# 10XGenomics/supernova

Measured on AMD Instinct MI355X. Metric: Gk-mers/s through count+graph at k=48, 1.2B×150bp; bit-exact counts, higher is better.
Workload: dtype u64

## Files before the change

### include/snk.h

```cpp
#ifndef SNK_H_
#define SNK_H_
#include <stddef.h>
#include <stdint.h>

#ifdef __cplusplus
extern "C" {
#endif

#define SNK_OK 0
#define SNK_E_ARG (-1)
#define SNK_E_HIP (-2)
#define SNK_E_NOGPU (-3)
#define SNK_E_NOMEM (-4)
#define SNK_E_IO (-5)
#define SNK_E_UNSUPPORTED (-6)
#define SNK_E_INTERNAL (-7)

typedef struct snk_ctx snk_ctx;

typedef struct snk_params {
    uint32_t K;
    uint32_t min_qual;
    uint32_t min_freq;
    uint32_t min_bc;
// ... 106 lines not shown
    const void* good_len;
    uint64_t n_kmers;
    const void* keys;
    const void* counts;
    const void* ctx;
    const void* spectrum;
    uint32_t spectrum_bins;
    uint32_t n_circles;
    uint64_t n_unitigs;
    uint64_t unitig_total_bases;
    const void* unitig_off;
    const void* unitig_bases;
    uint32_t rank_rounds;
    uint32_t buckets_split;
    uint32_t max_slots_used;
    uint32_t n_overflow;
    uint64_t scratch_bytes;
    float phase_ms[8];
    float kernel_ms[4];
    uint64_t n_boundary;
    uint64_t n_fragments;
    const void* unitig_group;
    float graph_ms[8];
    uint32_t repartitioned;
    uint32_t n_hot_buckets;
} snk_dev_result;

int snk_dev_count_graph(snk_ctx* ctx, const snk_dev_reads* in, const snk_params* p, snk_dev_result* out, void* stream,
                        char* err, size_t errcap);
int snk_dev_download(snk_ctx* ctx, const void* d_src, void* h_dst, size_t bytes, void* stream);

int snk_dev_stream_begin(snk_ctx* ctx, const snk_params* p, uint32_t read_len, uint64_t total_reads_ub, int has_bc, void* stream, char* err, size_t errcap);
int snk_dev_stream_append(snk_ctx* ctx, const snk_dev_reads* slab, void* stream, char* err, size_t errcap);
int snk_dev_stream_finish(snk_ctx* ctx, snk_dev_result* out, void* stream, char* err, size_t errcap);

uint64_t snk_pack2_bytes(uint64_t n_bases);
int snk_dev_pack2(snk_ctx* ctx, const void* d_bases, uint64_t n_bases, void* d_packed, void* stream);
int snk_dev_unpack2(snk_ctx* ctx, const void* d_packed, uint64_t n_bases, void* d_bases, void* stream);


typedef struct snk_comm snk_comm;
int snk_comm_set_rccl_path(const char* path);
int snk_comm_unique_id(void* id128, char* err, size_t errcap);
int snk_comm_create_rccl(snk_ctx* ctx, const void* id128, uint32_t rank, uint32_t world, snk_comm** out, char* err, size_t errcap);
int snk_comm_from_nccl(snk_ctx* ctx, void* nccl_comm, uint32_t rank, uint32_t world, snk_comm** out, char* err, size_t errcap);
int snk_comm_create_local(uint32_t world, snk_comm** out , char* err, size_t errcap);
typedef int (*snk_comm_a2a_fn)(void* user, const void* send, const uint64_t* sbeg, const uint64_t* scnt, void* recv, const uint64_t* rbeg,
                               const uint64_t* rcnt, uint32_t world);
typedef int (*snk_comm_gather_fn)(void* user, const void* mine, uint32_t k, unsigned long long* all, uint32_t world);
int snk_comm_create_callbacks(uint32_t rank, uint32_t world, snk_comm_a2a_fn a2a, snk_comm_gather_fn gather, void* user, snk_comm** out,
                              char* err, size_t errcap);
int snk_comm_selftest(snk_comm* c, uint64_t seed, uint32_t buckets_per_rank, uint32_t ranges, char* err, size_t errcap);
void snk_comm_destroy(snk_comm* c);
void snk_comm_abort(snk_comm* c);
uint32_t snk_comm_rank(const snk_comm* c);
uint32_t snk_comm_world(const snk_comm* c);
const char* snk_comm_kind(const snk_comm* c);

typedef struct snk_shard_result {
    uint32_t rank, world;
    uint64_t n_reads, n_instances, n_supermers, n_buckets_total;
    uint64_t n_kmers;
    const void* keys;
    const void* counts;
    const void* ctx;
    const void* spectrum;
    uint32_t spectrum_bins, n_circles;
    uint64_t n_unitigs, unitig_total_bases;
    const void* unitig_off;
    const void* unitig_bases;
    const void* unitig_circular;
    uint64_t n_frags, n_frags_total, n_queries, n_link_queries;
    uint64_t exchanged_bytes[8];
    uint32_t host_syncs;
    uint32_t ranking;
    uint32_t buckets_split, max_slots_used;
    float phase_ms[8];
    float join_ms[8];
    float count_kernel_ms;
    uint32_t repartitioned;
    uint32_t n_hot_buckets;
    uint32_t reserved_u;
    uint64_t pair_max_bytes[8];
} snk_shard_result;
uint32_t snk_ctx_last_partition_passes(const snk_ctx* ctx);
uint32_t snk_ctx_last_count_limit(const snk_ctx* ctx);
int snk_shard_step(snk_ctx* ctx, snk_comm* comm, const snk_dev_reads* in, const snk_params* p, uint64_t total_reads, uint32_t flags,
                   snk_shard_result* out, void* stream, char* err, size_t errcap);
int snk_shard_stream_begin(snk_ctx* ctx, snk_comm* comm, const snk_params* p, uint32_t read_len, uint64_t rank_reads_ub, uint64_t total_reads,
                           int has_bc, void* stream, char* err, size_t errcap);
int snk_shard_stream_append(snk_ctx* ctx, const snk_dev_reads* slab, void* stream, char* err, size_t errcap);
int snk_shard_stream_finish(snk_ctx* ctx, snk_comm* comm, uint32_t flags, snk_shard_result* out, void* stream, char* err, size_t errcap);
typedef struct snk_reads {
    uint64_t n_reads;
    uint32_t read_len;
    uint32_t reserved;
    const uint8_t* ascii;
    const uint32_t* rows;
    const uint16_t* lens;
    const uint8_t* quals;
    const uint16_t* good_len;
    const int32_t* bc;
    int64_t ign_bc_below;
} snk_reads;

typedef struct snk_result {
    uint64_t n_instances;
    uint64_t n_kmers;
    uint32_t* kmers;
    uint32_t* counts;
    uint8_t* ctx;
    uint64_t n_unitigs;
    uint64_t* unitig_off;
    uint8_t* unitig_bases;
    uint64_t* spectrum;
    uint32_t spectrum_bins;
    uint32_t reserved;
    float phase_ms[8];
    uint8_t* bv_image;
    uint64_t bv_bytes;
} snk_result;

int snk_count_graph(snk_ctx* ctx, const snk_reads* in, const snk_params* p, snk_result* out, char* err, size_t errcap);
void snk_free(snk_result* r);

int snk_shard_gather_unitigs(snk_ctx* ctx, snk_comm* comm, const snk_shard_result* res, uint32_t K, uint32_t root, uint32_t flags,
                             snk_result* out, void* stream, char* err, size_t errcap);

int snk_host_alloc_pinned(size_t bytes, void** out, char* err, size_t errcap);
void snk_host_free_pinned(void* p);

int snk_write_bv(const char* path, uint64_t n_unitigs, const uint64_t* unitig_off, const uint8_t* unitig_bases,
                 char* err, size_t errcap);
int snk_read_bv(const char* path, uint64_t* n_unitigs, uint64_t** unitig_off, uint8_t** unitig_bases, char* err,
                size_t errcap);

int snk_dev_bv_image(snk_ctx* ctx, uint32_t K, uint64_t n_unitigs, const void* d_unitig_off, const void* d_unitig_bases, int by_first_kmer,
                     const void** d_image, uint64_t* image_bytes, void* stream, char* err, size_t errcap);

typedef struct snk_hbv {
    int32_t n_vertices, n_edges;
    int32_t* v_left;
    int32_t* v_right;
    int32_t* src_unitig;
    uint8_t* is_rc;
    int32_t* fwd_xlat;
    int32_t* rev_xlat;
    int32_t* bvcomp_order;
} snk_hbv;
int snk_hbv_from_unitigs(uint32_t K, uint64_t n_unitigs, const uint64_t* unitig_off, const uint8_t* unitig_bases,
                         snk_hbv* out, char* err, size_t errcap);
uint32_t snk_ctx_last_hbv_flood(const snk_ctx* ctx, uint64_t* device_components, uint64_t* host_components);
uint32_t snk_ctx_last_local_graph(const snk_ctx* ctx, uint64_t* in_chunk_circles, uint32_t* big_chunks);
int snk_dev_hbv(snk_ctx* ctx, uint32_t K, uint64_t n_unitigs, const void* d_unitig_off, const void* d_unitig_bases,
                snk_hbv* out, float* device_ms, void* stream, char* err, size_t errcap);
void snk_hbv_free(snk_hbv* h);
typedef struct snk_dev_paths {
    uint64_t n_reads, n_edges_total;
    const void* offset;
    const void* n_edges;
    const void* start;
    const void* edges;
    uint64_t dict_slots;
    float dict_ms, path_ms;
    const void* unitig_bc_off;
    const void* unitig_bcs;
    uint64_t n_unitig_bcs;
    float bcs_ms;
    uint32_t lookup_index;
    uint64_t n_slow;
    uint32_t retries;
} snk_dev_paths;
#define SNK_PATH_UNITIG_BCS 1u
#define SNK_PATH_UNITIG_BCS_EXHAUSTIVE 2u
#define SNK_PATH_UNITIG_BCS_NOCUT 4u
int snk_dev_path_reads(snk_ctx* ctx, uint32_t K, const snk_dev_reads* in, uint64_t n_unitigs, const void* d_unitig_off, const void* d_unitig_bases,
                       const snk_hbv* h, snk_dev_paths* out, void* stream, char* err, size_t errcap);
int snk_dev_path_reads2(snk_ctx* ctx, uint32_t K, const snk_dev_reads* in, uint64_t n_unitigs, const void* d_unitig_off, const void* d_unitig_bases,
                        const snk_hbv* h, uint32_t flags, snk_dev_paths* out, void* stream, char* err, size_t errcap);
int snk_hbv_involution(const snk_hbv* h, uint64_t n_unitigs, int32_t* inv , char* err, size_t errcap);
int snk_write_hbv(const char* path_hbv, const char* path_inv, uint32_t K, uint64_t n_unitigs, const uint64_t* unitig_off,
                  const uint8_t* unitig_bases, const snk_hbv* h, char* err, size_t errcap);

typedef struct snk_dev_dups {
    uint64_t n_pairs;
    const void* dup;
    uint64_t n_placed;
    uint64_t n_dup_reads;
    uint64_t n_interdup_reads;
    uint64_t n_dup_pairs;
    uint64_t n_art_pairs;
    double interdup_rate;
    float ms;
} snk_dev_dups;
int snk_dev_mark_dups(snk_ctx* ctx, const snk_dev_reads* in, const snk_dev_paths* paths, snk_dev_dups* out, void* stream, char* err, size_t errcap);

typedef struct snk_dev_pidx {
    uint64_t n_hbv_edges, n_entries;
    const void* index_off;
    const void* index_ids;
    const void* counts;
    uint64_t n_empty_edges;
    float ms;
    uint32_t key_bits;
    uint64_t reserved[6];
} snk_dev_pidx;
int snk_dev_paths_index(snk_ctx* ctx, const snk_dev_paths* paths, uint64_t n_hbv_edges, const int32_t* inv, snk_dev_pidx* out, void* stream,
                        char* err, size_t errcap);
int snk_write_paths(const char* path, uint64_t n_reads, const int32_t* offset, const uint32_t* n_edges, const uint64_t* start, const int32_t* edges,
                    char* err, size_t errcap);
int snk_write_paths_index(const char* path_inv, const char* path_countsb, uint64_t n_hbv_edges, const uint64_t* index_off, const uint64_t* index_ids,
                          const int32_t* counts, char* err, size_t errcap);
int snk_write_dup(const char* path, uint64_t n_pairs, const uint8_t* dup, char* err, size_t errcap);

typedef struct snk_dev_pathsx {
    uint64_t n_reads, n_bytes, n_index;
    const void* data;
    const void* index;
    uint64_t n_empty;
    uint64_t n_steps_not_found;
    uint64_t n_offsets_wrapped;
    float ms;
    uint32_t reserved0;
    uint64_t reserved[6];
} snk_dev_pathsx;
int snk_dev_paths_zip(snk_ctx* ctx, const snk_dev_paths* paths, const snk_hbv* h, snk_dev_pathsx* out, void* stream, char* err, size_t errcap);
int snk_dev_paths_unzip(snk_ctx* ctx, const snk_dev_pathsx* in, const snk_hbv* h, snk_dev_paths* out, void* stream, char* err, size_t errcap);
int snk_write_pathsx(const char* path, uint64_t n_reads, const int64_t* index, uint64_t n_index, const uint8_t* data, uint64_t n_bytes, char* err, size_t errcap);
int snk_read_pathsx(const char* path, uint64_t* n_reads, uint64_t* n_index, int64_t** index, uint64_t* n_bytes, uint8_t** data, char* err, size_t errcap);
int snk_write_hbx(const char* path, uint32_t K, uint64_t n_unitigs, const uint64_t* unitig_off, const uint8_t* unitig_bases, const snk_hbv* h, char* err,
                  size_t errcap);

typedef struct snk_dev_extend {
    snk_dev_paths paths;
    uint64_t n_back_extended;
    uint64_t n_cut_to_first;
    uint64_t n_quality_extended;
    uint64_t n_ambiguous;
    uint64_t n_too_many;
    uint64_t n_exact_extended;
    float ms;
    uint32_t reserved0;
    uint64_t n_enumerated;
    uint64_t reserved[5];
} snk_dev_extend;
#define SNK_EXT_BACK 1u
int snk_dev_extend_paths(snk_ctx* ctx, uint32_t K, const snk_dev_reads* in, uint64_t n_unitigs, const void* d_unitig_off, const void* d_unitig_bases,
                         const snk_hbv* h, const snk_dev_paths* paths, uint32_t flags, snk_dev_extend* out, void* stream, char* err, size_t errcap);

#define SNK_BADS_X 1u
typedef struct snk_dev_bads {
    uint64_t n_pairs;
    const void* bad;
    uint64_t n_placed;
    uint64_t n_mismatch_reads;
    uint64_t n_bad_reads;
    uint64_t n_bad_pairs;
    uint64_t n_offsets_wrapped;
    float ms;
    uint32_t n_slabs;
    float tables_ms, kernel_ms;
    uint64_t reserved[5];
} snk_dev_bads;
int snk_dev_mark_bads(snk_ctx* ctx, uint32_t K, const snk_dev_reads* in, uint64_t n_unitigs, const void* d_unitig_off, const void* d_unitig_bases,
                      const snk_hbv* h, const snk_dev_paths* paths, uint32_t flags, snk_dev_bads* out, void* stream, char* err, size_t errcap);
struct snk_df_files;
int snk_dev_mark_bads_df(snk_ctx* ctx, uint32_t K, struct snk_df_files* f, uint64_t first, uint64_t n, uint32_t read_len, uint32_t threads, uint64_t slab_reads,
                         uint64_t n_unitigs, const void* d_unitig_off, const void* d_unitig_bases, const snk_hbv* h, const snk_dev_paths* paths, uint32_t flags,
                         snk_dev_bads* out, char* err, size_t errcap);

#define SNK_HOPS_ONE_GOOD 1u
#define SNK_HOPS_EXT_HOST 2u
typedef struct snk_dev_hops {
    uint64_t n_pairs;
    const void* pairs;
    uint64_t n_part1, n_part2, n_part3;
    uint64_t n_sink_edges;
    uint64_t n_long_edges;
    uint64_t n_two_class;
    uint64_t n_ext_round0;
    uint64_t n_ext_closure;
    uint64_t n_ext_host;
    uint64_t n_not_extended;
    float ms, tables_ms;
    uint32_t ext_budget;
    float part12_ms, part3_ms;
    uint64_t reserved[4];
} snk_dev_hops;
int snk_dev_edge_pairs(snk_ctx* ctx, uint32_t K, uint64_t n_unitigs, const void* d_unitig_off, const void* d_unitig_bases, const snk_hbv* h,
                       const int32_t* inv , const snk_dev_paths* paths, const snk_dev_pidx* px ,
                       const void* d_bc , const void* d_bad , uint32_t flags, uint32_t ext_budget ,
                       snk_dev_hops* out, void* stream, char* err, size_t errcap);
int snk_write_hops(const char* path, uint64_t n_pairs, const int32_t* pairs, char* err, size_t errcap);
int snk_read_hops(const char* path, uint64_t* n_pairs, int32_t** pairs, char* err, size_t errcap);

#define SNK_CLOSE_CG1 1u
#define SNK_CLOSE_PLACE_HOST 2u
typedef struct snk_dev_closures {
    uint64_t n_closures, n_bases, n_pairs;
    const void* closure_off;
    const void* bases;
    const void* pair_first;
    uint64_t n_pairs_0, n_pairs_1, n_pairs_2, n_pairs_many;
    uint64_t n_rows;
    uint64_t n_partners_tried, n_partners_placed;
    uint64_t n_followers;
// ... 267 lines not shown
```

### supernova_amd/csrc/snk_api.hip

```cpp
#include <math.h>
#include <stdlib.h>
#include <execinfo.h>
#include <dlfcn.h>
#include <time.h>

#include <algorithm>

#include "snk_ctx.h"
#include "snk_kernels.h"
#include "snk_synth.h"

static thread_local char g_last_error[512] = "";

hipError_t snk_enter(snk_ctx* ctx) { return hipSetDevice(ctx->device); }

void snk_set_mlen(snk_ctx* ctx, const snk_params* p) {
    uint32_t m = (p->flags & SNK_F_LONG_MINIMISER) ? (uint32_t)SNK_M_LONG : (uint32_t)SNK_M_OF(p->K);
    const unsigned long long v = snk_opt_u64(ctx, SNK_OPT_minimiser_len);
    if (v == SNK_M_LONG || v == SNK_M_OF(p->K)) m = (uint32_t)v;
    ctx->mlen = m;
}

void snk_set_error(char* err, size_t errcap, const char* fmt, ...) {
    va_list ap;
// ... 207 lines not shown
            ctx->total_alloc -= b;
            return true;
        }
    if (va_trace2()) fprintf(stderr, "[snk arena] R? %zu (not live)\n", off);
    return true;
}
}

static void arena_poison(void* p, size_t bytes) {
    static const bool on = getenv("SNK_ARENA_POISON") && *getenv("SNK_ARENA_POISON") == '1';
    if (on) { (void)hipMemset(p, 0xCD, bytes); (void)hipStreamSynchronize(nullptr); }
}

int snk_ctx_alloc(snk_ctx* ctx, size_t bytes, void** out, char* err, size_t errcap) {
    if (bytes == 0) bytes = 256;
    bytes = (bytes + 255) & ~(size_t)255;
    if (ctx->device_mem_total && bytes > 2 * ctx->device_mem_total) {
        void* fr[12];
        const int n = backtrace(fr, 12);
        Dl_info di;
        uintptr_t base = 0;
        if (dladdr((void*)&snk_ctx_alloc, &di) && di.dli_fbase) base = (uintptr_t)di.dli_fbase;
        char where[256];
        size_t w = 0;
        for (int i = 1; i < n && w + 20 < sizeof where; ++i) w += (size_t)snprintf(where + w, sizeof where - w, " +0x%zx", (size_t)((uintptr_t)fr[i] - base));
        return snk_fail(SNK_E_INTERNAL, err, errcap, "scratch request of %zu bytes (device: %zu) from libsnk%s", bytes, (size_t)ctx->device_mem_total, where);
    }
    if (ctx->va_state >= 0 && !ctx->arena_legacy) {
        if (void* q = va_alloc(ctx, bytes)) {
            ++ctx->alloc_serial;
            ctx->va_serial.push_back({(size_t)((char*)q - ctx->va_base), ctx->alloc_serial});
            ctx->total_alloc += bytes;
            if (ctx->total_alloc > ctx->peak_alloc) ctx->peak_alloc = ctx->total_alloc;
            *out = q;
            arena_poison(q, bytes);
            return SNK_OK;
        }
    }
    int best = -1;
    for (size_t i = 0; i < ctx->blocks.size(); ++i) {
        const snk_ctx::block& b = ctx->blocks[i];
        if (!b.used && b.bytes >= bytes && b.bytes <= 4 * bytes + (1u << 20) &&
            (best < 0 || b.bytes < ctx->blocks[best].bytes))
            best = (int)i;
    }
    if (best >= 0) {
        ctx->blocks[best].used = true;
        ctx->blocks[best].serial = ++ctx->alloc_serial;
        ctx->blocks[best].epoch = ctx->call_epoch;
        ctx->total_alloc += ctx->blocks[best].bytes;
        if (ctx->total_alloc > ctx->peak_alloc) ctx->peak_alloc = ctx->total_alloc;
        *out = ctx->blocks[best].p;
        arena_poison(*out, bytes);
        return SNK_OK;
    }
    void* p = nullptr;
    hipError_t e = hipMalloc(&p, bytes);
    if (e != hipSuccess) {
        (void)hipGetLastError();
        snk_ctx_trim_cache(ctx);
        e = hipMalloc(&p, bytes);
    }
    if (e != hipSuccess)
        return snk_fail(SNK_E_NOMEM, err, errcap, "hipMalloc(%zu) failed: %s", bytes, hipGetErrorString(e));
    ctx->blocks.push_back({p, bytes, true, ++ctx->alloc_serial, ctx->call_epoch});
    ctx->total_alloc += bytes;
    if (ctx->total_alloc > ctx->peak_alloc) ctx->peak_alloc = ctx->total_alloc;
    ctx->cached_bytes += bytes;
    *out = p;
    arena_poison(p, bytes);
    return SNK_OK;
}
static void release_poison(snk_ctx* ctx, const void* p, size_t bytes) {
    static const bool on = getenv("SNK_ARENA_POISON") && *getenv("SNK_ARENA_POISON") == '2';
    if (on && bytes) (void)hipMemsetAsync(const_cast<void*>(p), 0xDD, bytes, ctx->cur_stream ? ctx->cur_stream : ctx->stream);
}
void snk_ctx_release_block(snk_ctx* ctx, const void* p) {
    if (!p) return;
    if (ctx->va_state > 0 && (const char*)p >= ctx->va_base && (const char*)p < ctx->va_base + ctx->va_size) {
        const size_t off = (size_t)((const char*)p - ctx->va_base);
        for (auto& u : ctx->va_used) if (u.off == off) { release_poison(ctx, p, u.bytes); break; }
    }
    if (va_release(ctx, p)) return;
    for (auto& b : ctx->blocks)
        if (b.p == p && b.used) { release_poison(ctx, p, b.bytes); b.used = false; ctx->total_alloc -= b.bytes; return; }
}
void snk_ctx_release_since(snk_ctx* ctx, uint64_t mark, const void* const* keep, size_t n_keep) {
    if (ctx->va_state > 0) {
        std::vector<size_t> drop;
        for (auto& e : ctx->va_serial) {
            if (e.serial <= mark) continue;
            bool kept = false, live = false;
            for (size_t i = 0; i < n_keep; ++i) if (keep[i] == ctx->va_base + e.off) kept = true;
            for (auto& u : ctx->va_used) if (u.off == e.off) live = true;
            if (!kept && live) drop.push_back(e.off);
        }
        for (size_t off : drop) (void)va_release(ctx, ctx->va_base + off);
    }
    for (auto& b : ctx->blocks) {
        if (!b.used || b.serial <= mark) continue;
        bool kept = false;
        for (size_t i = 0; i < n_keep; ++i) if (keep[i] == b.p) kept = true;
        if (!kept) { b.used = false; ctx->total_alloc -= b.bytes; }
    }
}
void snk_ctx_release_scratch(snk_ctx* ctx) {
    if (ctx->stream_job && ctx->stream_job_invalidate) ctx->stream_job_invalidate(ctx->stream_job);
    if (ctx->shard) snk_shard_state_invalidate_job(ctx->shard);
    for (auto& b : ctx->blocks) b.used = false;
    ctx->total_alloc = 0;
    ctx->peak_alloc = 0;
    if (ctx->va_state > 0) {
        if (va_trace()) fprintf(stderr, "[snk arena] call done: mapped %.2f GB, high water %.2f GB, live ranges %zu, free ranges %zu\n", ctx->va_mapped / 1073741824.0,
                                ctx->va_high / 1073741824.0, ctx->va_used.size(), ctx->va_free.size());
        ctx->va_used.clear();
        ctx->va_serial.clear();
        ctx->va_free.clear();
        if (ctx->va_mapped) ctx->va_free.push_back(snk_ctx::vrange{0, ctx->va_mapped});
        const size_t recent = std::max(ctx->va_high, std::max(ctx->va_high_prev[0], ctx->va_high_prev[1]));
        ctx->va_high_prev[1] = ctx->va_high_prev[0];
        ctx->va_high_prev[0] = ctx->va_high;
        ctx->va_high = 0;
        const size_t floor_chunks = (ctx->va_floor + (((size_t)1 << 30) - 1)) & ~(((size_t)1 << 30) - 1);
        if (ctx->va_sealed || (recent && ctx->va_mapped > std::max(2 * recent + ((size_t)1 << 30), floor_chunks)) || (ctx->arena_legacy && ctx->va_mapped)) {
            va_reset(ctx);
            if (ctx->va_floor && !ctx->arena_legacy && ctx->va_state > 0) (void)va_grow(ctx, ctx->va_floor);
        }
        else if (ctx->va_floor > ctx->va_mapped && !ctx->arena_legacy && ctx->va_state > 0 && !ctx->va_sealed) (void)va_grow(ctx, ctx->va_floor - ctx->va_mapped);
    }
    ++ctx->call_epoch;
    bool stale = false;
    for (auto& b : ctx->blocks) if (b.epoch + 2 < ctx->call_epoch) stale = true;
    if (stale) {
        std::vector<snk_ctx::block> keep;
        for (auto& b : ctx->blocks) {
            if (b.epoch + 2 < ctx->call_epoch) { (void)hipFree(b.p); ctx->cached_bytes -= b.bytes; }
            else keep.push_back(b);
        }
        ctx->blocks.swap(keep);
    }
    snk_ctx_plan_mem(ctx);
}
extern "C" uint32_t snk_ctx_last_partition_passes(const snk_ctx* ctx) { return ctx ? ctx->last_partition_passes : 0u; }
extern "C" uint32_t snk_ctx_last_hbv_flood(const snk_ctx* ctx, uint64_t* device_components, uint64_t* host_components) {
    if (device_components) *device_components = ctx ? ctx->last_hbv_dev_components : 0;
    if (host_components) *host_components = ctx ? ctx->last_hbv_host_components : 0;
    return ctx ? ctx->last_hbv_flood : 0u;
}
extern "C" uint32_t snk_ctx_last_local_graph(const snk_ctx* ctx, uint64_t* in_chunk_circles, uint32_t* big_chunks) {
    if (in_chunk_circles) *in_chunk_circles = ctx ? ctx->last_bl_circles : 0;
    if (big_chunks) *big_chunks = ctx ? ctx->last_bl_big_chunks : 0u;
    return ctx ? ctx->last_bl_attempts : 0u;
}
extern "C" uint32_t snk_ctx_last_count_limit(const snk_ctx* ctx) { return ctx ? ctx->last_count_limit : 0u; }
extern "C" int snk_ctx_reserve(snk_ctx* ctx, uint64_t bytes, char* err, size_t errcap) {
    if (!ctx) return snk_fail(SNK_E_ARG, err, errcap, "snk_ctx_reserve: NULL context");
    SNK_HIP_TRY(snk_enter(ctx));
    if (!va_init(ctx)) return snk_fail(SNK_E_UNSUPPORTED, err, errcap, "snk_ctx_reserve: the growing arena is switched off (SNK_ARENA_VMM=0) or not available");
    if (ctx->va_sealed && ctx->va_used.empty()) va_reset(ctx);
    if (ctx->va_state <= 0) return snk_fail(SNK_E_UNSUPPORTED, err, errcap, "snk_ctx_reserve: no address range for the arena");
    if (bytes > ctx->va_mapped && !va_grow(ctx, bytes - ctx->va_mapped))
        return snk_fail(SNK_E_NOMEM, err, errcap, "snk_ctx_reserve: %.1f GB asked for, %.1f GB mapped", bytes / 1073741824.0, ctx->va_mapped / 1073741824.0);
    ctx->va_floor = bytes;
    return SNK_OK;
}
extern "C" void snk_ctx_trim(snk_ctx* ctx) {
    if (!ctx) return;
    ctx->va_floor = 0;
    (void)snk_enter(ctx);
    (void)hipDeviceSynchronize();
    snk_ctx_trim_cache(ctx);
}
void snk_ctx_plan_mem(snk_ctx* ctx) {
    size_t fr = 0, tot = 0;
    ctx->plan_mem = ctx->device_mem_total;
    ctx->plan_mapped = (uint64_t)ctx->cached_bytes;
    { const long long mb = (long long)snk_opt_u64(ctx, SNK_OPT_plan_mem_mb); if (mb > 0) { ctx->plan_mem = (uint64_t)mb << 20; return; } }
    if (hipMemGetInfo(&fr, &tot) != hipSuccess) { (void)hipGetLastError(); return; }
    uint64_t avail = (uint64_t)fr + (uint64_t)ctx->cached_bytes;
    avail &= ~((8ull << 30) - 1);
    if (avail < (8ull << 30)) avail = 8ull << 30;
    if (avail < ctx->plan_mem) ctx->plan_mem = avail;
}
void snk_ctx_trim_cache(snk_ctx* ctx) {
    if (ctx->va_state > 0) {
        size_t live_end = 0;
        for (auto& u : ctx->va_used) if (u.off + u.bytes > live_end) live_end = u.off + u.bytes;
        va_shrink(ctx, live_end);
    }
    std::vector<snk_ctx::block> keep;
    for (auto& b : ctx->blocks) {
        if (b.used) keep.push_back(b);
        else { (void)hipFree(b.p); ctx->cached_bytes -= b.bytes; }
    }
    ctx->blocks.swap(keep);
}

extern "C" void snk_ctx_destroy(snk_ctx* ctx) {
    if (!ctx) return;
    (void)snk_enter(ctx);
    snk_ctx_release_scratch(ctx);
    snk_ctx_trim_cache(ctx);
    if (ctx->va_base) { va_unmap_from(ctx, 0); (void)hipMemAddressFree(ctx->va_base, ctx->va_size); ctx->va_base = nullptr; }
    if (ctx->shard) snk_shard_state_free(ctx->shard);
    if (ctx->host_io && ctx->host_io_free) ctx->host_io_free(ctx->host_io);
    if (ctx->df_io && ctx->df_io_free) ctx->df_io_free(ctx->df_io);
    if (ctx->shard_host && ctx->shard_host_free) ctx->shard_host_free(ctx->shard_host);
    if (ctx->close_table && ctx->close_table_free) ctx->close_table_free(ctx->close_table);
    if (ctx->stream_job && ctx->stream_job_free) ctx->stream_job_free(ctx->stream_job);
    if (ctx->stream) (void)hipStreamDestroy(ctx->stream);
    delete ctx;
}

extern "C" void snk_synth_default(snk_synth_params* sp, uint64_t n_reads, uint64_t seed, int error_free) {
    memset(sp, 0, sizeof *sp);
    sp->seed = seed;
    sp->n_reads = n_reads;
    sp->read_len = 150;
    sp->genome_len = n_reads * 150 / 56;
    if (sp->genome_len < 1000) sp->genome_len = 1000;
    sp->mol_len = 50000;
    sp->mols_per_bc = 10;
    sp->pairs_per_bc = 400;
    sp->insert_min = 300;
    sp->insert_span = 101;
    sp->sub_ppm = error_free ? 0 : 2000;
    sp->unbarcoded_ppm = 20000;
    sp->lowq_tail_ppm = error_free ? 0 : 50000;
    sp->tail_max = 40;
    snk_synth_set_errors(sp, sp->sub_ppm);
}
extern "C" void snk_synth_set_errors(snk_synth_params* sp, uint32_t sub_ppm) {
    sp->sub_ppm = sub_ppm;
    double lam = sp->read_len * (double)sp->sub_ppm / 1e6, term = exp(-lam), cum = 0;
    for (int j = 0; j < 4; ++j) {
        cum += term;
        double v = cum * 4294967296.0;
        sp->err_cdf[j] = v >= 4294967295.0 ? 0xFFFFFFFFu : (uint32_t)v;
        term *= lam / (j + 1);
    }
}

extern "C" int snk_synth_host(const snk_synth_params* sp, uint64_t first, uint64_t n, uint32_t* rows, uint32_t row_words,
                              uint8_t* quals, uint32_t qstride, int32_t* bc) {
    if (!sp || sp->read_len == 0 || (rows && row_words * 16 < sp->read_len) || (quals && qstride < sp->read_len))
        return snk_fail(SNK_E_ARG, nullptr, 0, "snk_synth_host: bad arguments");
    for (uint64_t i = 0; i < n; ++i)
        snk_synth_read(*sp, first + i, rows ? rows + i * row_words : nullptr, row_words,
                       quals ? quals + i * (uint64_t)qstride : nullptr, bc ? bc + i : nullptr);
    return SNK_OK;
}

__global__ void __launch_bounds__(256) snk_synth_kernel(snk_synth_params sp, uint64_t first, uint64_t n, uint32_t* rows,
                                                        uint32_t row_words, uint8_t* quals, uint32_t qstride,
                                                        int32_t* bc) {
    uint64_t i = (uint64_t)blockIdx.x * blockDim.x + threadIdx.x;
    uint64_t step = (uint64_t)gridDim.x * blockDim.x;
    for (; i < n; i += step)
        snk_synth_read(sp, first + i, rows ? rows + i * row_words : nullptr, row_words,
                       quals ? quals + i * (uint64_t)qstride : nullptr, bc ? bc + i : nullptr);
}

extern "C" int snk_synth_dev(snk_ctx* ctx, const snk_synth_params* sp, uint64_t first, uint64_t n, void* d_rows,
                             uint32_t row_words, void* d_quals, uint32_t qstride, void* d_bc, void* stream) {
    char* err = nullptr;
    size_t errcap = 0;
    if (!ctx || !sp) return snk_fail(SNK_E_ARG, err, errcap, "snk_synth_dev: NULL ctx/params");
    if ((d_rows && row_words * 16 < sp->read_len) || (d_quals && qstride < sp->read_len))
        return snk_fail(SNK_E_ARG, err, errcap, "snk_synth_dev: row stride too small");
    if (n == 0) return SNK_OK;
    hipStream_t st = stream ? (hipStream_t)stream : ctx->stream;
    ctx->cur_stream = st;
    SNK_HIP_TRY(snk_launch(snk_synth_kernel, snk_blocks_capped(n, 256, 65536), 256, 0, st, *sp, first, n, (uint32_t*)d_rows, row_words,
                           (uint8_t*)d_quals, qstride, (int32_t*)d_bc));
    return SNK_OK;
}
```

### supernova_amd/csrc/snk_ctx.h

```cpp
#pragma once
#include <hip/hip_runtime.h>
#include <stdarg.h>
#include <stdio.h>
#include <string.h>

#include <initializer_list>
#include <string>
#include <vector>

#include "../../include/snk.h"
#include "snk_launch.h"
#include "snk_opts.h"
#include "snk_plan.h"

struct snk_ctx {
    int device = 0;
    hipStream_t stream = nullptr;
    hipStream_t cur_stream = nullptr;
    int n_cu = 256;
    size_t lds_per_block = 65536;
    uint64_t device_mem_total = 0;
    double pass_sigma = 0.0;
    uint64_t plan_mapped = 0;
    uint64_t plan_mem = 0;
    struct block { void* p; size_t bytes; bool used; uint64_t serial = 0; uint64_t epoch = 0; };
    uint64_t call_epoch = 0;
    uint64_t alloc_serial = 0;
    std::vector<block> blocks;
    struct vrange { size_t off, bytes; };
    char* va_base = nullptr;
    size_t va_size = 0, va_mapped = 0, va_high = 0, va_high_prev[2] = {0, 0};
    std::vector<hipMemGenericAllocationHandle_t> va_handles;
    std::vector<size_t> va_chunk;
    std::vector<vrange> va_free;
    std::vector<vrange> va_used;
    size_t va_floor = 0;
    int va_state = 0;
    bool va_sealed = false;
    struct vser { size_t off; uint64_t serial; };
    std::vector<vser> va_serial;
    bool arena_legacy = false;
    size_t total_alloc = 0;
    size_t peak_alloc = 0;
    size_t cached_bytes = 0;
    uint64_t last_n_kmers = 0, last_n_instances = 0;
    uint64_t last_region_max = 0, last_region_n = 0;
    uint64_t last_bnd = 0, last_bnd_n = 0;
    uint32_t last_ovf = 0, last_ovf_nb = 0;
    uint64_t last_ovf_reads = 0;
    uint64_t last_dense = 0;
    uint32_t count_screen = 0;
    uint32_t count_tight = 0;
    snk_sizing_history sizing;
    uint32_t mlen = 16;
    uint32_t last_extra = 0;
    uint64_t last_input_fp = 0;
    bool have_input_fp = false;
    uint32_t last_count_limit = 0;
    uint32_t last_partition_passes = 1;
    uint32_t last_hbv_flood = 0;
    uint64_t last_hbv_dev_components = 0, last_hbv_host_components = 0;
    uint32_t last_bl_attempts = 0, last_bl_big_chunks = 0;
    uint64_t last_bl_circles = 0;
    std::vector<unsigned long long> h_region_off;
    snk_opts opts;
    void* shard = nullptr;
    void* host_io = nullptr;
    void (*host_io_free)(void*) = nullptr;
    void* df_io = nullptr;
    void (*df_io_free)(void*) = nullptr;
    void* stream_job = nullptr;
    void (*stream_job_free)(void*) = nullptr;
    void (*stream_job_invalidate)(void*) = nullptr;
    void* shard_host = nullptr;
    void (*shard_host_free)(void*) = nullptr;
    void* close_table = nullptr;
    void (*close_table_free)(void*) = nullptr;
};

hipError_t snk_enter(snk_ctx* ctx);
void snk_set_error(char* err, size_t errcap, const char* fmt, ...);
void snk_set_mlen(snk_ctx* ctx, const snk_params* p);
hipError_t snk_sync_at(hipStream_t st, const char* file, int line);
uint64_t snk_sync_count();
#define snk_sync(st) snk_sync_at((st), __FILE__, __LINE__)
int snk_fail(int code, char* err, size_t errcap, const char* fmt, ...);

#define SNK_HIP_TRY(expr)                                                                          \
    do {                                                                                           \
        hipError_t _e = (expr);                                                                    \
        if (_e != hipSuccess)                                                                      \
            return snk_fail(_e == hipErrorOutOfMemory ? SNK_E_NOMEM : SNK_E_HIP, err, errcap,      \
                            "%s failed: %s (%s:%d)", #expr, hipGetErrorString(_e), __FILE__, __LINE__); \
    } while (0)

int snk_ctx_alloc(snk_ctx* ctx, size_t bytes, void** out, char* err, size_t errcap);
void snk_ctx_release_scratch(snk_ctx* ctx);
void snk_ctx_release_block(snk_ctx* ctx, const void* p);
void snk_ctx_release_since(snk_ctx* ctx, uint64_t mark, const void* const* keep, size_t n_keep);
void snk_ctx_trim_cache(snk_ctx* ctx);
void snk_ctx_plan_mem(snk_ctx* ctx);

struct snk_dev_owner {
    snk_ctx* ctx;
    hipStream_t st;
    std::vector<void*> mine;
    snk_dev_owner(snk_ctx* c, hipStream_t s) : ctx(c), st(s) {}
    snk_dev_owner(const snk_dev_owner&) = delete;
    snk_dev_owner& operator=(const snk_dev_owner&) = delete;
    ~snk_dev_owner() {
        if (st) (void)hipStreamSynchronize(st);
        for (void* p : mine) (void)hipFree(p);
        if (st && ctx->cur_stream == st) ctx->cur_stream = nullptr;
    }
    template <typename T>
    hipError_t alloc(T** out, size_t bytes) {
        mine.reserve(mine.size() + 1);
        void* p = nullptr;
        const hipError_t e = hipMalloc(&p, bytes);
        if (e == hipSuccess) mine.push_back(p);
        *out = (T*)p;
        return e;
    }
    void keep(std::initializer_list<const void*> ps) {
        for (const void* p : ps)
            for (void*& m : mine)
                if (m == p) m = nullptr;
    }
};

void snk_shard_state_free(void* p);
void snk_shard_state_invalidate_job(void* p);
```

### supernova_amd/csrc/snk_dist.hip

```cpp
#include <string.h>

#include <vector>

#include "snk_ctx.h"
#include "snk_common.h"
#include "snk_graph.h"
#include "snk_kernels.h"
#include "snk_stages.h"
#include "snk_shard.h"

void snk_shard_state_free(void* p) { delete static_cast<snk_shard_state*>(p); }
void snk_shard_state_invalidate_job(void* p) { if (p) static_cast<snk_shard_state*>(p)->job_open = false; }

static snk_shard_state* step_reset(snk_ctx* ctx, const snk_params* p, uint32_t rank, uint32_t world, uint32_t NB_total) {
    snk_ctx_release_scratch(ctx);
    snk_shard_state* S = snk_shard_state_of(ctx);
    S->params = *p;
    S->rank = rank; S->world = world; S->NB_total = NB_total; S->NBl = NB_total / world;
    S->circ_all = nullptr; S->join_circles = 0;
    ctx->last_bl_attempts = ctx->last_bl_big_chunks = 0; ctx->last_bl_circles = 0;
    return S;
}

static const char* const BEGIN_WHO = "snk_shard_hist";
int snk_shard_begin(snk_ctx* ctx, const snk_dev_reads* in, const snk_params* p, uint32_t rank, uint32_t world, uint32_t NB_total,
                    uint64_t* n_instances, hipStream_t st, char* err, size_t errcap) {
    if (!ctx || !in || !p) return snk_fail(SNK_E_ARG, err, errcap, "%s: NULL argument", BEGIN_WHO);
    int rc;
    if ((rc = snk_intake_check_params(p, err, errcap))) return rc;
    if (world == 0 || rank >= world || NB_total == 0 || NB_total % world) return snk_fail(SNK_E_ARG, err, errcap, "%s: NB_total must be a positive multiple of world", BEGIN_WHO);
    if (world > 0x7FFF) return snk_fail(SNK_E_UNSUPPORTED, err, errcap, "world > 32767");
    if (snk_intake_reads_fault(in)) return snk_fail(SNK_E_ARG, err, errcap, "%s: bad reads", BEGIN_WHO);
    SNK_HIP_TRY(snk_enter(ctx));
    snk_shard_state* S = step_reset(ctx, p, rank, world, NB_total);
    const uint16_t* good_len;
    snk_fused_trim ft;
    bool fused;
    if ((rc = snk_intake_trim(ctx, st, in, p, &good_len, &ft, &fused, err, errcap))) return rc;
    if ((rc = snk_intake_status(ctx, st, &S->status, err, errcap))) return rc;
    unsigned long long h_plan[2] = {0, 0};
    unsigned long long* d_plan = nullptr;
    if (!fused && (rc = snk_stage_partition_plan(ctx, st, p->K, good_len, in->n_reads, h_plan, err, errcap, &d_plan))) return rc;
    const unsigned long long kpr = in->read_len >= p->K ? in->read_len - p->K + 1 : 0;
    if ((rc = snk_stage_partition(ctx, st, p->K, in, good_len, NB_total, in->n_reads * kpr, in->n_reads, false, S->status, &S->part, err, errcap, d_plan, h_plan,
                                  fused ? &ft : nullptr))) return rc;
    if (n_instances) *n_instances = h_plan[0];
    return SNK_OK;
}

int snk_shard_job_open(snk_ctx* ctx, const snk_params* p, uint32_t rank, uint32_t world, uint32_t NB_total, uint32_t read_len, uint64_t reads_ub,
                       uint64_t total_reads, int has_bc, hipStream_t st, char* err, size_t errcap) {
    if (!ctx || !p) return snk_fail(SNK_E_ARG, err, errcap, "snk_shard_stream_begin: NULL argument");
    int rc;
    if ((rc = snk_intake_check_params(p, err, errcap))) return rc;
    if (world == 0 || rank >= world || NB_total == 0 || NB_total % world) return snk_fail(SNK_E_ARG, err, errcap, "snk_shard_stream_begin: NB_total must be a positive multiple of world");
    if (read_len == 0 || read_len > 256 || reads_ub == 0) return snk_fail(SNK_E_ARG, err, errcap, "snk_shard_stream_begin: read_len 1..256 and an upper bound of this rank's reads are needed");
    SNK_HIP_TRY(snk_enter(ctx));
    snk_shard_state* S = step_reset(ctx, p, rank, world, NB_total);
    S->job_open = false; S->job_read_len = read_len; S->job_has_bc = has_bc; S->job_reads_ub = reads_ub; S->job_total_reads = total_reads;
    if ((rc = snk_intake_status(ctx, st, &S->status, err, errcap))) return rc;
    void* q;
    if ((rc = snk_ctx_alloc(ctx, reads_ub * 2 + 64, &q, err, errcap))) return rc; S->job_good_len = (uint16_t*)q;
    const unsigned long long kpr = read_len >= p->K ? read_len - p->K + 1 : 0;
    if ((rc = snk_partition_open(ctx, st, p->K, NB_total, reads_ub * kpr, reads_ub, false, S->status, &S->job, err, errcap))) return rc;
    S->job_open = true;
    return SNK_OK;
}
int snk_shard_job_add(snk_ctx* ctx, const snk_dev_reads* slab, hipStream_t st, char* err, size_t errcap) {
    if (!ctx || !ctx->shard || !slab) return snk_fail(SNK_E_ARG, err, errcap, "snk_shard_stream_append: NULL argument / no open step");
    snk_shard_state* S = snk_shard_state_of(ctx);
    if (!S->job_open) return snk_fail(SNK_E_ARG, err, errcap, "snk_shard_stream_append: no open step (snk_shard_stream_begin)");
    if (slab->n_reads == 0) return SNK_OK;
    int rc = snk_intake_check_slab(slab, S->job_read_len, S->job_has_bc != 0, S->job.n_reads, S->job_reads_ub, "snk_shard_stream_append", "step's", "rank's", err, errcap);
    if (rc) return rc;
    SNK_HIP_TRY(snk_enter(ctx));
    return snk_intake_add_slab(ctx, st, &S->job, slab, S->params.min_qual, S->job_good_len + S->job.n_reads, err, errcap);
}
int snk_shard_job_adopt(snk_ctx* ctx, uint64_t* n_instances, hipStream_t st, char* err, size_t errcap) {
    snk_shard_state* S = snk_shard_state_of(ctx);
    if (!S->job_open) return snk_fail(SNK_E_ARG, err, errcap, "snk_shard_stream_finish: no open step");
    S->job_open = false;
    unsigned long long h_plan[2] = {0, 0};
    int rc = snk_partition_close(ctx, st, &S->job, &S->part, h_plan, err, errcap);
    if (rc) return rc;
    if (n_instances) *n_instances = h_plan[0];
    return SNK_OK;
}

int snk_shard_prune_plan(snk_ctx* ctx, snk_shard_state& S, hipStream_t st, char* err, size_t errcap) {
    snk_bl_state& B = S.bl;
    memset(&B, 0, sizeof B);
    B.tab = &S.tab;
    B.K = S.params.K; B.rank = S.rank; B.world = S.world; B.NB_total = S.NB_total; B.NBl = S.NBl;
    B.do_prune = S.params.min_freq > 1 ? 1u : 0u;
    int rc = snk_bl_dist_plan(ctx, st, &B, err, errcap);
    if (rc) return rc;
    snk_dist_graph& g = S.g;
    memset(&g, 0, sizeof g);
    g.K = B.K; g.rank = B.rank; g.world = B.world; g.NB_total = B.NB_total; g.NBl = B.NBl; g.do_prune = B.do_prune;
    g.n = S.tab.n; g.keys = S.tab.keys; g.vals = S.tab.vals;
    g.index = B.index; g.index_mask = B.index_mask;
    g.ctx = B.ctx; g.counts = B.counts; g.rq_idx = B.rq_idx; g.rq_meta = B.rq_meta;
    return SNK_OK;
}

namespace {
constexpr unsigned long long RT_RC = 1ull, RT_CIRC = 2ull, RT_HEAD = 4ull;
__device__ __forceinline__ uint32_t owner_of_frag(const unsigned long long* __restrict__ frag_off, uint32_t world, unsigned long long g) {
    uint32_t r = 0;
    while (r + 1 < world && g >= frag_off[r + 1]) ++r;
    return r;
}
constexpr int ROUTE_TILES = 16;
template <bool FILL>
__global__ void __launch_bounds__(256) route_kernel(uint64_t Fl, unsigned long long f0, const uint32_t* __restrict__ nk, const uint32_t* __restrict__ pl_pid,
                                                    const unsigned long long* __restrict__ pl_koff, const unsigned long long* __restrict__ pl_N,
                                                    const uint8_t* __restrict__ pl_circ, const unsigned long long* __restrict__ frag_off, uint32_t world,
                                                    uint32_t K, const uint64_t* __restrict__ boff, const uint8_t* __restrict__ bases,
                                                    unsigned long long* __restrict__ cnt_or_cur , unsigned long long* __restrict__ hdr,
                                                    uint8_t* __restrict__ bout, const unsigned long long* __restrict__ base_seg ) {
    extern __shared__ unsigned long long dynr[];
    __shared__ unsigned long long c_src[256], c_dst[256];
    __shared__ uint32_t c_len[256];
    unsigned long long* lfr = dynr;
    unsigned long long* lby = dynr + world;
    unsigned long long* cfr = dynr + 2 * world;
    unsigned long long* cby = dynr + 3 * world;
    for (uint32_t r = threadIdx.x; r < 4 * world; r += 256) dynr[r] = 0;
    __syncthreads();
    const uint64_t fbase = (uint64_t)blockIdx.x * 256 * ROUTE_TILES + threadIdx.x;
    for (int t = 0; t < ROUTE_TILES; ++t) {
        const uint64_t f = fbase + (uint64_t)t * 256;
        if (f < Fl) {
            const uint32_t owner = owner_of_frag(frag_off, world, pl_pid[f] >> 1);
            atomicAdd(&lfr[owner], 1ull);
            atomicAdd(&lby[owner], (unsigned long long)((uint64_t)nk[f] + K - 1));
        }
    }
    __syncthreads();
    for (uint32_t r = threadIdx.x; r < world; r += 256) {
        const unsigned long long cf = lfr[r], cb = lby[r];
        if (cf) {
            const unsigned long long a = atomicAdd(&cnt_or_cur[r], cf), b = atomicAdd(&cnt_or_cur[world + r], cb);
            lfr[r] = a; lby[r] = b;
        }
    }
    if (!FILL) return;
    for (int t = 0; t < ROUTE_TILES; ++t) {
        __syncthreads();
        const uint64_t f = fbase + (uint64_t)t * 256;
        c_len[threadIdx.x] = 0;
        if (f < Fl) {
            const uint32_t pid = pl_pid[f];
            const uint32_t owner = owner_of_frag(frag_off, world, pid >> 1);
            const uint64_t len = (uint64_t)nk[f] + K - 1;
            const unsigned long long slot = lfr[owner] + atomicAdd(&cfr[owner], 1ull), bo = lby[owner] + atomicAdd(&cby[owner], (unsigned long long)len);
            const unsigned long long ko = pl_koff[f];
            const unsigned long long g = f0 + f;
            const bool head = (ko & ~(1ull << 63)) == 0 && (pid >> 1) == (uint32_t)g;
            const unsigned long long flags = ((ko >> 63) ? RT_RC : 0ull) | (pl_circ[f] ? RT_CIRC : 0ull) | (head ? RT_HEAD : 0ull);
            hdr[4 * slot + 0] = (unsigned long long)pid | (g << 32);
            hdr[4 * slot + 1] = (unsigned long long)nk[f] | (flags << 32);
            hdr[4 * slot + 2] = head ? pl_N[f] : (ko & ~(1ull << 63));
            hdr[4 * slot + 3] = bo - base_seg[owner];
            c_src[threadIdx.x] = boff[f];
            c_dst[threadIdx.x] = bo;
            c_len[threadIdx.x] = (uint32_t)len;
        }
        __syncthreads();
        const uint32_t sub = threadIdx.x & 7u;
        for (uint32_t i = threadIdx.x >> 3; i < 256; i += 32) {
            const uint32_t n = c_len[i];
            const uint8_t* src = bases + c_src[i];
// ... 172 lines not shown
```

### supernova_amd/csrc/snk_graph.h

```cpp
#pragma once
#include <rocprim/rocprim.hpp>

#include "snk_ctx.h"
#include "snk_kernels.h"

#define G_ALLOC(ptr, type, count)                                                       \
    do {                                                                                \
        void* _p = nullptr;                                                             \
        int _rc = snk_ctx_alloc(ctx, sizeof(type) * (size_t)(count), &_p, err, errcap); \
        if (_rc) return _rc;                                                            \
        ptr = (type*)_p;                                                                \
    } while (0)

template <typename T, typename In>
static int excl_scan(snk_ctx* ctx, hipStream_t st, In in, T* out, size_t count, char* err, size_t errcap) {
    size_t tb = 0;
    SNK_HIP_TRY(rocprim::exclusive_scan((void*)nullptr, tb, in, out, (T)0, count, rocprim::plus<T>(), st));
    void* tmp;
    int rc = snk_ctx_alloc(ctx, tb, &tmp, err, errcap);
    if (rc) return rc;
    SNK_HIP_TRY(rocprim::exclusive_scan(tmp, tb, in, out, (T)0, count, rocprim::plus<T>(), st));
    return SNK_OK;
}

struct snk_graph_out {
    uint8_t* ctx;
    uint32_t* counts;
    unsigned long long* spectrum;
    uint32_t spectrum_bins;
    uint64_t n_unitigs;
    uint64_t total_bases;
    uint64_t* unitig_off;
    uint8_t* unitig_bases;
    uint32_t* unitig_group;
    uint32_t n_circles;
    uint32_t rank_rounds;
    uint64_t n_boundary;
    uint64_t n_fragments;
};

int snk_graph_sort(snk_ctx* ctx, hipStream_t st, uint32_t K, uint64_t n, snk_u128* keys_in, uint64_t* vals_in,
                   snk_u128* keys_out, uint64_t* vals_out, char* err, size_t errcap);
int snk_graph_build(snk_ctx* ctx, hipStream_t st, uint32_t K, const snk_u128* keys, const uint64_t* vals, uint64_t n,
                    uint32_t do_prune, bool want_unitigs, snk_graph_out* out, char* err, size_t errcap);

struct snk_dist_graph {
    uint32_t K, rank, world, NB_total, NBl, do_prune;
    uint64_t n;
    const snk_u128* keys;
    const uint64_t* vals;
    unsigned long long* index;
    uint64_t index_mask;
    uint8_t* ctx;
    uint32_t* counts;
    uint32_t* rq_idx;
    uint16_t* rq_meta;
};
struct snk_frag_out {
    uint64_t n_frags, total_bases;
    uint32_t* nk;
    unsigned long long* hl_self;
    unsigned long long* hl_nb;
    uint64_t* boff;
    uint8_t* bases;
    unsigned long long* spectrum;
    uint32_t spectrum_bins, n_circles, rank_rounds;
    uint32_t* fgroup;
    uint32_t* sfrag;
    uint32_t n_local_circles;
};
struct snk_join_out {
    uint64_t n_unitigs, total_bases;
    uint64_t* unitig_off;
    uint8_t* unitig_bases;
    uint8_t* unitig_circular;
    uint32_t* unitig_group;
    uint32_t n_circles, rank_rounds;
};
struct snk_placement {
    uint32_t* pid;
    unsigned long long* koff;
    unsigned long long* N;
    uint8_t* circ;
};
struct snk_rank_trace;
int snk_join_rank(snk_ctx* ctx, hipStream_t st, uint64_t F, const uint32_t* nk, uint32_t* flink, const uint2** rk_out, uint8_t** circ_out,
                  uint32_t* n_circles, uint32_t* rounds, char* err, size_t errcap, uint8_t* circ_given = nullptr,
                  snk_rank_trace* trace = nullptr );
int snk_join_place(snk_ctx* ctx, hipStream_t st, const uint2* rk, const uint32_t* nk, const uint8_t* circ, uint64_t f0, uint64_t Fl,
                   snk_placement* pl, char* err, size_t errcap, uint64_t rk_f0 = 0);
int snk_join_emit(snk_ctx* ctx, hipStream_t st, uint32_t K, uint64_t F, const uint32_t* nk, const uint32_t* gfid, const uint32_t* pl_pid,
                  const unsigned long long* pl_koff, const unsigned long long* pl_N, const uint8_t* pl_circ, uint32_t pid_base, uint64_t n_pid,
                  const uint64_t* boff, const uint8_t* fbases, const uint32_t* fgroup, snk_join_out* out, char* err, size_t errcap);
int snk_dist_answer(snk_ctx* ctx, hipStream_t st, snk_dist_graph* g, const void* d_queries, uint64_t nq, void* d_ans, char* err,
                    size_t errcap);
int snk_dist_apply(snk_ctx* ctx, hipStream_t st, snk_dist_graph* g, const void* d_qbuf, const void* d_ans, uint64_t nq,
                   const unsigned long long* d_qoff, char* err, size_t errcap);
int snk_dist_join(snk_ctx* ctx, hipStream_t st, uint32_t K, uint64_t F, const uint32_t* nk, const unsigned long long* hl_self,
                  const unsigned long long* hl_nb, const uint64_t* boff, const uint8_t* fbases, uint64_t total_fbases,
                  snk_join_out* out, char* err, size_t errcap, const uint32_t* fgroup = nullptr, const uint32_t* sfrag = nullptr,
                  uint64_t n_states = 0);
int snk_dist_links_query(snk_ctx* ctx, hipStream_t st, const snk_frag_out* fr, const unsigned long long* d_node_off, uint32_t world,
                         unsigned long long my_end_base, unsigned long long* d_cursor, void* d_qbuf, char* err, size_t errcap);
int snk_dist_links_answer(snk_ctx* ctx, hipStream_t st, const snk_frag_out* fr, const void* d_queries, uint64_t nq, unsigned long long my_state_base,
                          uint64_t n_local_states, unsigned long long my_end_base, void* d_ans, char* err, size_t errcap);
int snk_dist_links_apply_regions(snk_ctx* ctx, hipStream_t st, const snk_frag_out* fr, const void* d_qbuf, const void* d_ans, uint32_t world, uint64_t cap,
                                 const unsigned long long* counts, uint32_t** flink_out, char* err, size_t errcap);

struct snk_table;
struct snk_bl_state {
    const snk_table* tab;
    uint32_t K, rank, world, NB_total, NBl, do_prune, force_dist;
    uint4* desc;
    uint32_t nchunks, nbig;
    uint32_t* biglist;
    uint8_t *ctx, *pend, *premote;
    uint32_t *counts, *nbr, *rq;
    uint32_t* rq_idx;
    uint16_t* rq_meta;
    unsigned long long* index;
    uint64_t index_mask, n_boundary;
    unsigned long long *qcount, *qcursor;
    unsigned long long* spec;
    uint32_t want_spec, spec_over;
};
int snk_bl_dist_plan(snk_ctx* ctx, hipStream_t st, snk_bl_state* B, char* err, size_t errcap);
int snk_bl_dist_fill(snk_ctx* ctx, hipStream_t st, snk_bl_state* B, const unsigned long long* d_qoff, void* d_qbuf, char* err, size_t errcap);
int snk_bl_dist_fragments(snk_ctx* ctx, hipStream_t st, snk_bl_state* B, const unsigned long long* d_node_off, unsigned long long my_node_off,
                          snk_frag_out* out, char* err, size_t errcap);
int snk_local_graph(snk_ctx* ctx, hipStream_t st, uint32_t K, const snk_table* tab, uint32_t do_prune, bool want_unitigs,
                    bool sort_table, bool grouped, snk_graph_out* out, snk_u128** keys_final, float* ms , char* err,
                    size_t errcap);
int snk_spectrum(snk_ctx* ctx, hipStream_t st, const uint32_t* counts, uint64_t n, unsigned long long** bins_out, uint32_t* nbins_out,
                 char* err, size_t errcap);
```

### supernova_amd/csrc/snk_local.hip

```cpp
#include <string.h>
#include <cstring>
#include <rocprim/rocprim.hpp>

#include <type_traits>

#include "snk_ctx.h"
#include "snk_common.h"
#include "snk_kernels.h"
#include "snk_graph.h"
#include "snk_stages.h"

namespace {

constexpr uint32_t NONE = 0xFFFFFFFFu;
constexpr unsigned long long NONE64 = ~0ull;
constexpr uint16_t NONE16 = 0xFFFFu;
constexpr int TB = 256;

struct chunk_src {
    const uint32_t* chunk_n;
    const uint32_t* chunk_base;
    const uint4* extra;
    const unsigned long long* region_off;
    uint32_t NB, n_extra, n_regions;
    const uint8_t* span;
};
struct chunk_t {
    uint32_t bucket, n, lg, id;
    uint32_t span;
    uint64_t base;
};
struct bl_regions {
    const snk_u128* keys_r;
    const uint64_t* vals_r;
    const uint64_t* desc_src;
    snk_u128* keys_dense;
};
struct bl_shard {
    uint32_t bucket_base, NBl, me;
    uint32_t G;
    uint8_t* premote;
};
__global__ void __launch_bounds__(256) bl_chunk_merge_kernel(const uint32_t* __restrict__ chunk_n, const uint32_t* __restrict__ chunk_base, uint32_t NB, uint32_t G,
                                                             uint32_t cap, uint8_t* __restrict__ span, uint32_t* __restrict__ merged) {
    const uint32_t r = blockIdx.x * 256 + threadIdx.x;
    if (r >= G) return;
    uint32_t head = NONE, total = 0, m = 0, expect = 0;
    for (uint32_t b = r; b < NB; b += G) {
        const uint32_t n = chunk_n[b];
        span[b] = 1;
        merged[b] = n;
        if (n == 0) { head = NONE; continue; }
        const uint32_t base = chunk_base[b];
        if (head != NONE && base == expect && total + n <= cap && m < 255u) {
            total += n; ++m;
            merged[head] = total; merged[b] = 0; span[head] = (uint8_t)m;
        } else { head = b; total = n; m = 1; }
        expect = base + n;
    }
}
__global__ void __launch_bounds__(256) bl_chunk_desc_kernel(chunk_src cs, uint32_t nchunks, uint4* __restrict__ desc, uint64_t region_cap, uint64_t* __restrict__ desc_src) {
    const uint32_t c = blockIdx.x * 256 + threadIdx.x;
    if (c >= nchunks) return;
    uint32_t bucket, n, off = 0, meta = 0, region;
    if (c < cs.NB) {
        bucket = c; n = cs.chunk_n[c];
        if (n) off = cs.chunk_base[c];
        region = bucket % cs.n_regions;
        if (cs.span && n && cs.span[c] > 1) meta = 0x80000000u | cs.span[c];
    } else {
        const uint4 e = cs.extra[c - cs.NB];
        bucket = e.x; off = e.y; n = e.z & 0xFFFu; region = e.z >> 12; meta = e.w;
    }
    const uint64_t base = cs.region_off[region] + off;
    desc[c] = make_uint4((uint32_t)base, n, bucket, meta);
    if (desc_src) desc_src[c] = (uint64_t)region * region_cap + off;
}
__device__ __forceinline__ chunk_t chunk_get(const uint4* __restrict__ desc, uint32_t c) {
    const uint4 d = desc[c];
    chunk_t k;
    k.base = d.x; k.n = d.y; k.bucket = d.z; k.lg = d.w >> 24; k.id = d.w & 0xFFFFFFu; k.span = 1;
    if (d.w >> 31) { k.lg = 0; k.id = 0; k.span = d.w & 0xFFFFu; }
    return k;
}

__device__ __forceinline__ snk_kmer load_key(const snk_u128* keys, uint64_t i) {
    const uint64_t* p = reinterpret_cast<const uint64_t*>(keys + i);
    snk_kmer k;
    k.lo = p[0];
    k.hi = p[1];
    return k;
}
__device__ __forceinline__ uint32_t lhash(uint64_t hi, uint64_t lo) {
    uint32_t x = (uint32_t)(hi >> 32) * 0x9E3779B1u ^ (uint32_t)hi * 0x85EBCA77u ^ (uint32_t)(lo >> 32) * 0xC2B2AE3Du ^
                 (uint32_t)lo * 0x27D4EB2Fu;
    return snk_mix32(x);
}
template <int K>
__device__ __forceinline__ uint32_t oriented_base(snk_kmer k, bool rc, int idx) {
    return rc ? (snk_kmer_base<K>(k, K - 1 - idx) ^ 3u) : snk_kmer_base<K>(k, idx);
}

constexpr int BL_SPEC_LDS = 128;
constexpr int BL_SPEC_REPL = 64;
constexpr uint32_t BL_SPEC_BINS = 65536u;
constexpr uint32_t BL_SPEC_OVER = BL_SPEC_BINS + BL_SPEC_REPL * BL_SPEC_LDS / 2;
constexpr uint32_t BL_SPEC_WORDS = BL_SPEC_OVER + 16;
__global__ void __launch_bounds__(BL_SPEC_LDS) bl_spec_fold_kernel(unsigned long long* __restrict__ spec) {
    const uint32_t* rep = reinterpret_cast<const uint32_t*>(spec + BL_SPEC_BINS);
    unsigned long long s = 0;
    for (int r = 0; r < BL_SPEC_REPL; ++r) s += rep[r * BL_SPEC_LDS + threadIdx.x];
    spec[threadIdx.x] += s;
}
template <int K, int CAP, int T, bool BIG, bool GR, int MM>
__device__ __forceinline__ void bl_prune_chunk(const uint32_t c, const uint4* __restrict__ desc, uint32_t NB, bl_shard sh, const bl_regions& rg,
                                                     const snk_u128* __restrict__ keys, const uint64_t* __restrict__ vals,
                                                     uint32_t do_prune, uint8_t* __restrict__ ctx_out,
                                                     uint32_t* __restrict__ count_out, uint8_t* __restrict__ pend_out,
                                                     uint32_t* __restrict__ nbr_out, uint32_t* __restrict__ nbnd,
                                                     uint32_t* __restrict__ biglist, uint32_t* __restrict__ nbig,
                                                     unsigned long long* __restrict__ gindex, uint64_t gmask,
                                                     unsigned long long* __restrict__ spec, uint32_t* __restrict__ shist) {
    constexpr int HT = CAP <= 256 ? 512 : 4096;
    typedef typename std::conditional<(K <= 48 && !GR), uint32_t, uint64_t>::type klo_w;
    constexpr int KLS = (K <= 48 && !GR) ? 32 : 0;
    constexpr bool ONE = !BIG && T == 64;
    constexpr int ML = ONE ? 128 : 8 * T;
    __shared__ uint64_t khi[CAP];
    __shared__ klo_w klo[CAP];
    __shared__ uint32_t ht[ONE ? HT / 2 : HT];
    __shared__ uint32_t bcnt;
    const int tid = threadIdx.x;
    const chunk_t ch = chunk_get(desc, c);
    if (ch.n == 0) return;
    if (!BIG && ch.n > (uint32_t)CAP) {
        if (tid == 0) biglist[atomicAdd(nbig, 1u)] = c;
        return;
    }
    const uint32_t n = ch.n;
    uint64_t src = ch.base;
    if (rg.keys_r) { src = rg.desc_src[c]; keys = rg.keys_r; vals = rg.vals_r; }
    __syncthreads();
    for (int s = tid; s < (ONE ? HT / 2 : HT); s += T) ht[s] = 0;
    if constexpr (!ONE) { if (tid == 0) bcnt = 0; }
    constexpr int NPT = (CAP + T - 1) / T;
    {
        snk_kmer kq[NPT];
#pragma unroll
        for (int q = 0; q < NPT; ++q) {
            const uint32_t i = tid + q * T;
            if (i < n) kq[q] = load_key(keys, src + i);
        }
#pragma unroll
        for (int q = 0; q < NPT; ++q) {
            const uint32_t i = tid + q * T;
            if (i < n) {
                khi[i] = kq[q].hi;
                klo[i] = (klo_w)(kq[q].lo >> KLS);
                if (rg.keys_r) { uint64_t* d = reinterpret_cast<uint64_t*>(rg.keys_dense + ch.base + i); d[0] = kq[q].lo; d[1] = kq[q].hi; }
            }
        }
    }
    uint64_t vnext = (uint32_t)tid < n ? vals[src + tid] : 0ull;
    __syncthreads();
    for (uint32_t i = tid; i < n; i += T) {
        uint32_t slot = lhash(khi[i], (uint64_t)klo[i] << KLS) & (HT - 1);
        if constexpr (ONE) {
            for (;;) {
                uint32_t* const w = &ht[slot >> 1];
                const uint32_t s16 = (slot & 1u) << 4;
                const uint32_t cur = *reinterpret_cast<volatile uint32_t*>(w);
                if ((cur >> s16) & 0xFFFFu) { slot = (slot + 1) & (HT - 1); continue; }
                if (atomicCAS(w, cur, cur | ((i + 1u) << s16)) == cur) break;
            }
        } else {
            for (;;) {
                const uint32_t old = atomicCAS(&ht[slot], 0u, i + 1u);
                if (old == 0u) break;
                slot = (slot + 1) & (HT - 1);
            }
        }
    }
    __syncthreads();
    const uint32_t split_mask = (1u << ch.lg) - 1u;
    uint32_t mybnd = 0;
    __shared__ uint16_t mlist[ML];
    __shared__ uint32_t resL[T];
    __shared__ uint32_t mcnt;
    const uint16_t* const ht16 = reinterpret_cast<const uint16_t*>(ht);
    for (uint32_t i0 = 0; i0 < n; i0 += T) {
        const uint32_t i = i0 + tid;
        const bool act = i < n;
        snk_kmer k;
        k.hi = act ? khi[i] : 0ull;
        k.lo = act ? ((uint64_t)klo[i] << KLS) : 0ull;
        uint64_t tag = 0;
        if (GR) { tag = k.lo & 0xFFFFFFFFull; k.lo &= ~0xFFFFFFFFull; }
        const uint64_t v = vnext;
        vnext = i + T < n ? vals[src + i + T] : 0ull;
        const uint32_t c0 = (uint32_t)(v & 0xFFu);
        uint32_t keep = 0, miss = 0, nb0 = NONE, nb1 = NONE;
        const snk_kmer kr = snk_kmer_rc<K>(k);
        for (uint32_t rem = c0; rem; rem &= rem - 1) {
            const uint32_t bit = __ffs(rem) - 1;
            const snk_kmer y = bit < 4 ? snk_kmer_succ<K>(k, bit) : snk_kmer_pred<K>(k, bit - 4);
            const snk_kmer r = bit < 4 ? snk_kmer_pred<K>(kr, 3u - bit) : snk_kmer_succ<K>(kr, 7u - bit);
            const bool rev = snk_kmer_lt(r, y);
            snk_kmer cy = rev ? r : y;
            if (GR) cy.lo |= tag;
            int32_t j = -1;
            uint32_t slot = lhash(cy.hi, cy.lo) & (HT - 1);
            for (;;) {
                const uint32_t e = ONE ? (uint32_t)ht16[slot] : ht[slot];
                if (e == 0u) break;
                if (khi[e - 1] == cy.hi && ((uint64_t)klo[e - 1] << KLS) == cy.lo) { j = (int32_t)(e - 1); break; }
                slot = (slot + 1) & (HT - 1);
            }
            if (j >= 0) {
                keep |= 1u << bit;
                if (bit < 4) nb0 = ((uint32_t)j << 1) | (rev ? 1u : 0u); else nb1 = ((uint32_t)j << 1) | (rev ? 1u : 0u);
            } else miss |= 1u << bit;
        }
        if constexpr (!ONE) { if (tid == 0) mcnt = 0; }
        resL[tid] = 0;
        __syncthreads();
        const uint32_t nmiss = (uint32_t)__popc(miss);
        uint32_t pos, total = 0;
        if constexpr (ONE) {
            const uint32_t incl = snk_wave_scan_incl(nmiss);
            total = (uint32_t)__builtin_amdgcn_readlane((int)incl, 63);
            pos = incl - nmiss;
        } else pos = snk_wave_alloc(&mcnt, nmiss);
        constexpr int SH = K - MM;
        constexpr int PER = (SH + 3) / 4;
        for (uint32_t base = 0;; base += ML) {
            {
                uint32_t e = pos - base;
                for (uint32_t rem = miss; rem; rem &= rem - 1, ++e)
                    if (e < (uint32_t)ML) mlist[e] = (uint16_t)((tid << 3) | (__ffs(rem) - 1));
            }
            __syncthreads();
            if constexpr (!ONE) total = mcnt;
            const uint32_t nm = total - base < (uint32_t)ML ? total - base : (uint32_t)ML;
            for (uint32_t it0 = 0; it0 < nm; it0 += T / 4) {
                const uint32_t item = it0 + (tid >> 2), sub = tid & 3u;
                const bool on = item < nm;
                const uint32_t ent = on ? mlist[item] : 0u;
                const uint32_t th = ent >> 3, bit = ent & 7u;
                const uint32_t ni = i0 + th;
                snk_kmer kk;
                kk.hi = on ? khi[ni] : 0ull;
                kk.lo = on ? ((uint64_t)klo[ni] << KLS) : 0ull;
                uint64_t ktag = 0;
                if (GR) { ktag = kk.lo & 0xFFFFFFFFull; kk.lo &= ~0xFFFFFFFFull; }
                const int first = bit < 4 ? 1 : 0;
                uint32_t mk = 0xFFFFFFFFu;
                for (int t = 0; t < PER; ++t) {
                    const int sp = (int)sub * PER + t;
                    if (sp < SH) {
                        const int pp = first + sp;
                        uint64_t w;
                        if (pp == 0) w = kk.hi;
                        else if (pp < 32) w = (kk.hi << (2 * pp)) | (kk.lo >> (64 - 2 * pp));
                        else if (pp == 32) w = kk.lo;
                        else w = kk.lo << (2 * pp - 64);
                        const uint32_t key = snk_mmer_key_top<MM>(w);
                        mk = key < mk ? key : mk;
                    }
                }
                { const uint32_t o = __shfl_xor(mk, 1); mk = o < mk ? o : mk; }
                { const uint32_t o = __shfl_xor(mk, 2); mk = o < mk ? o : mk; }
                if (on && sub == 0) {
                    const snk_kmer y = bit < 4 ? snk_kmer_succ<K>(kk, bit) : snk_kmer_pred<K>(kk, bit - 4);
                    uint64_t wn;
                    if (bit < 4) {
                        constexpr int pl = K - MM;
                        wn = pl < 32 ? ((y.hi << (2 * pl)) | (y.lo >> (64 - 2 * pl))) : (pl == 32 ? y.lo : (y.lo << (2 * pl - 64)));
                    } else wn = y.hi;
                    const uint32_t nkey = snk_mmer_key_top<MM>(wn);
                    if (nkey < mk) mk = nkey;
                    const uint32_t gb = snk_bucket_of_key(mk ^ (GR ? snk_group_mix((uint32_t)ktag) : 0u), NB);
                    const uint32_t db = gb - (sh.bucket_base + ch.bucket);
                    bool here = ch.span == 1 ? db == 0u : (gb >= sh.bucket_base + ch.bucket && db % sh.G == 0u && db / sh.G < ch.span);
                    const bool remote = sh.NBl && gb / sh.NBl != sh.me;
                    if (here && ch.lg) {
                        const snk_kmer r = snk_kmer_rc<K>(y);
                        snk_kmer cn = snk_kmer_lt(r, y) ? r : y;
                        if (GR) cn.lo |= ktag;
                        uint32_t h1, h2;
                        snk_kmer_hash_count<(K > 48) || GR>(cn, &h1, &h2);
                        here = (h2 & split_mask) == ch.id;
                    }
                    if (here && !(do_prune & 2u)) { if (!(do_prune & 1u)) atomicOr(&resL[th], 1u << bit); }
                    else atomicOr(&resL[th], (1u << bit) | (0x100u << bit) | (remote ? (0x10000u << bit) : 0u));
                }
            }
            if (base + ML >= total) break;
            __syncthreads();
        }
        __syncthreads();
        const uint32_t res = resL[tid];
        keep |= res & 0xFFu;
        const uint32_t pm = (res >> 8) & 0xFFu;
        __syncthreads();
        if (!act) continue;
        const uint64_t gi = ch.base + i;
        ctx_out[gi] = (uint8_t)keep;
        pend_out[gi] = (uint8_t)pm;
        if (sh.premote) sh.premote[gi] = (uint8_t)(res >> 16);
        const uint32_t cnt = (uint32_t)(v >> 8);
        count_out[gi] = cnt;
        if (spec) {
            const uint32_t sc = cnt > 0xFFFFFFu ? 0xFFFFFFu : cnt;
            if (sc < (uint32_t)BL_SPEC_LDS) atomicAdd(&shist[sc], 1u);
            else if (sc < BL_SPEC_BINS) atomicAdd(&spec[sc], 1ull);
            else spec[BL_SPEC_OVER] = 1ull;
        }
        nbr_out[gi] = (nb0 == NONE ? 0x0FFFu : nb0) | (snk_kmer_eq(k, kr) ? 0x8000u : 0u) | ((nb1 == NONE ? 0x0FFFu : nb1) << 16);
        if (pm) {
            ++mybnd;
            if (gindex) {
                snk_kmer kk;
                kk.hi = khi[i];
                kk.lo = (uint64_t)klo[i] << KLS;
                uint32_t h1, h2;
                snk_kmer_hash2(kk, &h1, &h2);
                uint64_t slot = (((uint64_t)h1 << 32) | h2) & gmask;
                const unsigned long long ent = ((unsigned long long)h1 << 32) | (unsigned long long)(gi + 1);
                if (gindex[gmask + 1] == 0ull) {
                    bool placed = false;
                    for (uint32_t tries = 0; tries < 64; ++tries) {
                        const unsigned long long old = atomicCAS(&gindex[slot], 0ull, ent);
                        if (old == 0ull) { placed = true; break; }
                        slot = (slot + 1) & gmask;
                    }
                    if (!placed) gindex[gmask + 1] = 1ull;
                }
            }
        }
    }
    if constexpr (ONE) {
        const uint32_t b = (uint32_t)__builtin_amdgcn_readlane((int)snk_wave_scan_incl(mybnd), 63);
        if (tid == 0) nbnd[c] = b;
    } else {
        snk_wave_add(&bcnt, mybnd);
        __syncthreads();
        if (tid == 0) nbnd[c] = bcnt;
    }
}
template <int K, bool BIG, bool GR, int MM>
constexpr int bl_prune_waves = BIG ? 1 : (K <= 48 && !GR) ? (MM <= 16 ? 8 : 7) : 6;
template <int K, int CAP, int T, bool BIG, bool GR, int MM>
__global__ void __launch_bounds__(T) __attribute__((amdgpu_waves_per_eu(bl_prune_waves<K, BIG, GR, MM>, 8))) bl_prune_kernel(const uint4* __restrict__ desc, uint32_t NB, bl_shard sh, bl_regions rg, const uint32_t* __restrict__ biglist_in,
                                                     uint32_t nchunks, uint32_t cpw,
                                                     const snk_u128* __restrict__ keys, const uint64_t* __restrict__ vals,
                                                     uint32_t do_prune, uint8_t* __restrict__ ctx_out,
                                                     uint32_t* __restrict__ count_out, uint8_t* __restrict__ pend_out,
                                                     uint32_t* __restrict__ nbr_out, uint32_t* __restrict__ nbnd,
                                                     uint32_t* __restrict__ biglist, uint32_t* __restrict__ nbig, const uint32_t* __restrict__ n_dev,
                                                     unsigned long long* __restrict__ gindex, uint64_t gmask, unsigned long long* __restrict__ spec) {
    __shared__ uint32_t shist[BL_SPEC_LDS];
    if (spec) {
        for (int j = threadIdx.x; j < BL_SPEC_LDS; j += T) shist[j] = 0;
        __syncthreads();
    }
    if (BIG && n_dev) {
        const uint32_t nb = *n_dev;
        for (uint32_t w = blockIdx.x; w < nb; w += gridDim.x)
            bl_prune_chunk<K, CAP, T, BIG, GR, MM>(biglist_in[w], desc, NB, sh, rg, keys, vals, do_prune, ctx_out, count_out, pend_out, nbr_out, nbnd, biglist, nbig, gindex, gmask,
                                                   spec, shist);
    } else {
        for (uint32_t r = 0; r < cpw; ++r) {
            const uint32_t w = blockIdx.x * cpw + r;
            if (w >= nchunks) break;
            bl_prune_chunk<K, CAP, T, BIG, GR, MM>(BIG ? biglist_in[w] : w, desc, NB, sh, rg, keys, vals, do_prune, ctx_out, count_out, pend_out, nbr_out,
                                           nbnd, biglist, nbig, gindex, gmask, spec, shist);
        }
    }
    if (spec) {
        __syncthreads();
        uint32_t* rep = reinterpret_cast<uint32_t*>(spec + BL_SPEC_BINS) + (blockIdx.x % BL_SPEC_REPL) * BL_SPEC_LDS;
        for (int j = threadIdx.x; j < BL_SPEC_LDS; j += T)
            if (shist[j]) atomicAdd(&rep[j], shist[j]);
    }
}

__global__ void __launch_bounds__(TB) bl_index_build_kernel(const snk_u128* __restrict__ keys, const uint8_t* __restrict__ pend,
                                                            uint64_t n, unsigned long long* __restrict__ tab, uint64_t mask) {
    const uint64_t i = (uint64_t)blockIdx.x * TB + threadIdx.x;
    if (i >= n || !pend[i]) return;
    const snk_kmer k = load_key(keys, i);
    uint32_t h1, h2;
    snk_kmer_hash2(k, &h1, &h2);
    uint64_t slot = (((uint64_t)h1 << 32) | h2) & mask;
    const unsigned long long ent = ((unsigned long long)h1 << 32) | (unsigned long long)(i + 1);
    for (;;) {
        const unsigned long long old = atomicCAS(&tab[slot], 0ull, ent);
        if (old == 0ull) break;
        slot = (slot + 1) & mask;
    }
}
template <int K, bool GR>
__global__ void __launch_bounds__(TB) bl_resolve_kernel(const snk_u128* __restrict__ keys, const uint8_t* __restrict__ pend,
                                                        uint64_t n, const unsigned long long* __restrict__ tab, uint64_t mask,
                                                        uint32_t do_prune, uint8_t* __restrict__ ctx, uint32_t* __restrict__ rq,
                                                        const uint8_t* __restrict__ premote) {
    constexpr int SPAN = 8 * TB;
    __shared__ uint16_t list[SPAN];
    __shared__ uint32_t cnt;
    const uint64_t base = (uint64_t)blockIdx.x * SPAN;
    if (threadIdx.x == 0) cnt = 0;
    __syncthreads();
    {
        const uint64_t i8 = base + 8ull * threadIdx.x;
        unsigned long long w = 0;
        if (i8 + 8 <= n) w = *reinterpret_cast<const unsigned long long*>(pend + i8);
        else for (uint64_t q = i8; q < n; ++q) w |= (unsigned long long)pend[q] << (8 * (q - i8));
        if (w) {
            uint32_t m = 0;
            for (int q = 0; q < 8; ++q) if ((w >> (8 * q)) & 0xFFull) ++m;
            uint32_t pos = atomicAdd(&cnt, m);
            for (int q = 0; q < 8; ++q) if ((w >> (8 * q)) & 0xFFull) list[pos++] = (uint16_t)(8 * threadIdx.x + q);
        }
    }
    __syncthreads();
    const uint32_t m = cnt;
    for (uint32_t it = threadIdx.x; it < m; it += TB) {
        const uint64_t i = base + list[it];
        const uint32_t pm = pend[i] & (premote ? ~(uint32_t)premote[i] : 0xFFu);
        snk_kmer k = load_key(keys, i);
        uint64_t tag = 0;
        if (GR) { tag = k.lo & 0xFFFFFFFFull; k.lo &= ~0xFFFFFFFFull; }
        uint32_t c = ctx[i];
        const snk_kmer kr = snk_kmer_rc<K>(k);
        for (uint32_t rem = pm; rem; rem &= rem - 1) {
            const uint32_t bit = __ffs(rem) - 1;
            const snk_kmer y = bit < 4 ? snk_kmer_succ<K>(k, bit) : snk_kmer_pred<K>(k, bit - 4);
            const snk_kmer r = bit < 4 ? snk_kmer_pred<K>(kr, 3u - bit) : snk_kmer_succ<K>(kr, 7u - bit);
            const bool rev = snk_kmer_lt(r, y);
            snk_kmer cy = rev ? r : y;
            if (GR) cy.lo |= tag;
            uint32_t h1, h2;
            snk_kmer_hash2(cy, &h1, &h2);
            uint64_t slot = (((uint64_t)h1 << 32) | h2) & mask;
            int64_t j = -1;
            for (;;) {
                const unsigned long long e = tab[slot];
                if (e == 0ull) break;
                if ((uint32_t)(e >> 32) == h1) {
                    const uint64_t idx = (uint32_t)e - 1u;
                    if (snk_kmer_eq(load_key(keys, idx), cy)) { j = (int64_t)idx; break; }
                }
                slot = (slot + 1) & mask;
            }
            if (j >= 0) rq[2 * i + (bit >> 2)] = ((uint32_t)j << 1) | (rev ? 1u : 0u);
            else if (do_prune) c &= ~(1u << bit);
            else rq[2 * i + (bit >> 2)] = NONE;
        }
        ctx[i] = (uint8_t)c;
    }
}

struct bl_extra_pool {
    unsigned long long* cur;
    uint64_t f0, b0;
    uint64_t fcap, bcap;
};
struct bl_dist_args {
    const uint8_t* premote;
    const uint32_t* rq_idx;
    const uint16_t* rq_meta;
    const unsigned long long* node_off;
    unsigned long long my_node_off;
};
template <int K, int CAP, int T, bool BIG, bool EMIT, bool DIST, bool GR>
__global__ void __launch_bounds__(T) bl_frag_kernel(const uint4* __restrict__ desc, const uint32_t* __restrict__ biglist_in,
                                                    const snk_u128* __restrict__ keys, const uint8_t* __restrict__ ctx,
                                                    const uint8_t* __restrict__ pend, const uint32_t* __restrict__ nbr,
                                                    const uint32_t* __restrict__ rq, bl_dist_args da, uint32_t* __restrict__ nfrag,
                                                    const uint32_t* __restrict__ foff, const uint64_t* __restrict__ boff,
                                                    uint32_t* __restrict__ nk, unsigned long long* __restrict__ hl_self,
                                                    unsigned long long* __restrict__ hl_nb, uint64_t* __restrict__ bstart,
                                                    uint8_t* __restrict__ fbases, uint32_t* __restrict__ fgroup, uint32_t* __restrict__ sfrag, bl_extra_pool xp) {
    constexpr int SPT = (2 * CAP + T - 1) / T;
    constexpr int NPT = (CAP + T - 1) / T;
    constexpr bool ONEW = T == 64;
    typedef typename std::conditional<(K <= 48 && !GR), uint32_t, uint64_t>::type klo_w;
    constexpr int KLS = (K <= 48 && !GR) ? 32 : 0;
    __shared__ uint64_t khi[ONEW ? 1 : CAP];
    __shared__ klo_w klo[ONEW ? 1 : CAP];
    __shared__ uint16_t nbL[2 * CAP];
    typedef typename std::conditional<(CAP <= 256), uint32_t, uint64_t>::type wrec_t;
    constexpr int FB = CAP <= 256 ? 10 : 16;
    constexpr uint32_t FM = (1u << FB) - 1u;
    __shared__ uint16_t lnk[2 * CAP];
    __shared__ wrec_t wr[2 * CAP];
    constexpr bool WIDE = (uint32_t)CAP * (uint32_t)K > 65535u;
    uint16_t* foffL = nbL;
    __shared__ uint32_t frel[WIDE ? CAP : 1];
    __shared__ uint16_t hnode[CAP];
    __shared__ uint8_t ctxL[CAP], pendL[CAP];
    __shared__ uint32_t fcnt, bcnt, changed;
    const int tid = threadIdx.x;
    const uint32_t c = BIG ? biglist_in[blockIdx.x] : blockIdx.x;
    const chunk_t ch = chunk_get(desc, c);
    if (ch.n == 0) return;
    if (!BIG && ch.n > (uint32_t)CAP) return;
    const uint32_t n = ch.n;
    const uint32_t c_foff = EMIT ? foff[c] : 0u;
    const uint64_t c_boff = EMIT ? boff[c] : 0ull;
    if constexpr (!ONEW) {
        if (tid == 0) { fcnt = 0; bcnt = 0; changed = 0; }
    }
    uint32_t w_frags = 0, w_bases = 0;
    snk_kmer kq[NPT] = {};
    {
        uint32_t cq[NPT], pq[NPT];
        uint32_t nq[NPT];
#pragma unroll
        for (int q = 0; q < NPT; ++q) {
            const uint32_t i = tid + q * T;
            if (i < n) {
                const uint64_t gi = ch.base + i;
                if (EMIT) kq[q] = load_key(keys, gi);
                cq[q] = ctx[gi];
                pq[q] = pend[gi];
                nq[q] = nbr[gi];
            }
        }
#pragma unroll
        for (int q = 0; q < NPT; ++q) {
            const uint32_t i = tid + q * T;
            if (i < n) {
                if constexpr (EMIT && !ONEW) {
                    const snk_kmer k = kq[q];
                    khi[i] = k.hi;
                    klo[i] = (klo_w)(k.lo >> KLS);
                }
                ctxL[i] = (uint8_t)cq[q];
                pendL[i] = (uint8_t)pq[q];
                nbL[2 * i] = (uint16_t)(nq[q] & 0x8FFFu);
                nbL[2 * i + 1] = (uint16_t)((nq[q] >> 16) & 0x0FFFu);
            }
        }
    }
    __syncthreads();
    auto is_pal = [&](uint32_t i) -> bool { return (nbL[2 * i] >> 15) != 0; };
    auto key_of = [&](uint32_t i) -> snk_kmer {
        snk_kmer k;
        if constexpr (ONEW) {
            k = load_key(keys, ch.base + i);
            k.lo = (k.lo >> KLS) << KLS;
        } else {
            k.hi = khi[i];
            k.lo = (uint64_t)klo[i] << KLS;
        }
        return k;
    };
    auto own_key = [&](int q, uint32_t i) -> snk_kmer {
        if constexpr (ONEW) return kq[q];
        else return key_of(i);
    };
    uint32_t myterm = 0;
    for (uint32_t s = tid; s < 2 * n; s += T) {
        const uint32_t i = s >> 1, side = s & 1u;
        const uint32_t cc = ctxL[i];
        const uint32_t bits = side ? (cc >> 4) : (cc & 15u);
        uint16_t out = NONE16;
        if (__popc(bits) == 1) {
            const uint32_t b = __ffs(bits) - 1;
            if (!((pendL[i] >> (4 * side + b)) & 1u)) {
                const uint32_t nb = nbL[s] & 0x0FFFu;
                if (nb != 0x0FFFu) {
                    const uint32_t j = nb >> 1, rev = nb & 1u;
                    const uint32_t fs = side ^ 1u ^ rev;
                    const uint32_t cj = ctxL[j];
                    const uint32_t deg = fs ? __popc(cj & 0xF0u) : __popc(cj & 0x0Fu);
                    if (deg == 1 && !is_pal(i) && !is_pal(j)) out = (uint16_t)((j << 1) | fs);
                }
            }
        }
        lnk[s] = out;
        if (!EMIT) { if (out == NONE16) ++myterm; }
        else if (out == NONE16) wr[s] = (wrec_t)FM | ((wrec_t)s << (2 * FB));
        else wr[s] = (wrec_t)(out ^ 1u) | ((wrec_t)1 << FB) | ((wrec_t)(out ^ 1u) << (2 * FB));
    }
    if (!EMIT) {
        if constexpr (ONEW) {
            const uint32_t total = (uint32_t)__builtin_amdgcn_readlane((int)snk_wave_scan_incl(myterm), 63);
            if (tid == 0) nfrag[c] = total >> 1;
        } else {
            snk_wave_add(&fcnt, myterm);
            __syncthreads();
            if (tid == 0) nfrag[c] = fcnt >> 1;
        }
        return;
    }
    __syncthreads();
    int max_rounds = 2;
    while ((1u << (max_rounds - 1)) < 2 * n) ++max_rounds;
    for (int round = 0; round < max_rounds; ++round) {
        wrec_t rr[SPT];
        bool any = false;
#pragma unroll
        for (int q = 0; q < SPT; ++q) {
            if ((uint32_t)(q * T) >= 2 * n) break;
            const uint32_t s = tid + q * T;
            if (s < 2 * n) {
                const wrec_t a0 = wr[s];
                const uint32_t n1 = (uint32_t)a0 & FM;
                rr[q] = a0;
                if (n1 != FM) {
                    const wrec_t a1 = wr[n1];
                    const uint32_t d = (((uint32_t)(a0 >> FB) & FM) + ((uint32_t)(a1 >> FB) & FM)) & FM;
                    rr[q] = (a1 & (wrec_t)FM) | ((wrec_t)d << FB) | (a1 & ((wrec_t)FM << (2 * FB)));
                    any = true;
                }
            }
        }
        if constexpr (ONEW) {
            if (!__any(any)) break;
        }
        __syncthreads();
#pragma unroll
        for (int q = 0; q < SPT; ++q) {
            if ((uint32_t)(q * T) >= 2 * n) break;
            const uint32_t s = tid + q * T;
            if (s < 2 * n) wr[s] = rr[q];
        }
        if constexpr (ONEW) {
            __syncthreads();
        } else {
            if (any) changed = 1;
            __syncthreads();
            const bool go = changed != 0;
            __syncthreads();
            if (tid == 0) changed = 0;
            if (!go) break;
        }
    }
    __syncthreads();
    auto w_next = [&](uint32_t st) -> uint32_t { return (uint32_t)wr[st] & FM; };
    auto w_dist = [&](uint32_t st) -> uint32_t { return (uint32_t)(wr[st] >> FB) & FM; };
    auto w_tail = [&](uint32_t st) -> uint32_t { return (uint32_t)(wr[st] >> (2 * FB)) & FM; };

    auto half_link = [&](uint32_t s) -> unsigned long long {
        const uint32_t i = s >> 1, side = s & 1u;
        const uint32_t cc = ctxL[i];
        const uint32_t bits = side ? (cc >> 4) : (cc & 15u);
        if (__popc(bits) != 1 || is_pal(i)) return NONE64;
        const uint32_t b = __ffs(bits) - 1;
        if (!((pendL[i] >> (4 * side + b)) & 1u)) return NONE64;
        snk_kmer k = key_of(i);
        if (GR) k.lo &= ~0xFFFFFFFFull;
        const snk_kmer y = side ? snk_kmer_pred<K>(k, b) : snk_kmer_succ<K>(k, b);
        if (snk_kmer_eq(y, snk_kmer_rc<K>(y))) return NONE64;
        const uint64_t gi = ch.base + i;
        if (DIST && ((da.premote[gi] >> (4 * side + b)) & 1u)) {
            const uint32_t a = da.rq_idx[2 * gi + side];
            if (a == NONE) return NONE64;
            const uint32_t meta = da.rq_meta[2 * gi + side];
            const uint32_t fs = side ^ 1u ^ (meta >> 15);
            return 2ull * (da.node_off[meta & 0x7FFFu] + a) + fs;
        }
        const uint32_t a = rq[2 * gi + side];
        if (a == NONE) return NONE64;
        const uint32_t rev = a & 1u, fs = side ^ 1u ^ rev;
        return 2ull * ((DIST ? da.my_node_off : 0ull) + (a >> 1)) + fs;
    };
    auto describe = [&](uint32_t lf, uint32_t rel, uint32_t pid, uint32_t other, uint32_t cnt, uint32_t head_node, bool head_rc, uint32_t group) {
        const uint64_t f = (uint64_t)c_foff + lf;
        nk[f] = cnt;
        hl_self[2 * f] = 2ull * ((DIST ? da.my_node_off : 0ull) + ch.base) + pid;
        hl_self[2 * f + 1] = 2ull * ((DIST ? da.my_node_off : 0ull) + ch.base) + other;
        hl_nb[2 * f] = half_link(pid);
        hl_nb[2 * f + 1] = half_link(other);
        bstart[f] = c_boff + rel;
        if (sfrag) { sfrag[2 * ch.base + pid] = (uint32_t)(2 * f); sfrag[2 * ch.base + other] = (uint32_t)(2 * f + 1); }
        if (GR) fgroup[f] = group;
        if constexpr (WIDE) { foffL[pid] = (uint16_t)lf; frel[lf] = rel; }
        else foffL[pid] = (uint16_t)rel;
        hnode[lf] = (uint16_t)((head_node << 1) | (head_rc ? 1u : 0u));
    };

#pragma unroll
    for (int q = 0; q < NPT; ++q) {
        if ((uint32_t)(q * T) >= n) break;
        const uint32_t i = tid + q * T;
        bool head = false, fwd = false;
        uint32_t tR = 0, tL = 0, cnt = 0;
        if (i < n && w_next(2 * i) == FM) {
            tR = w_tail(2 * i); tL = w_tail(2 * i + 1);
            const uint32_t dR = w_dist(2 * i), dL = w_dist(2 * i + 1);
            fwd = tL < tR;
            head = (fwd ? dL : dR) == 0;
            cnt = dR + dL + 1u;
        }
        const uint32_t nb = head ? cnt + (uint32_t)K - 1u : 0u;
        uint32_t lf = 0, rel = 0;
        if constexpr (ONEW) {
            const unsigned long long hm = __ballot(head);
            if (hm == 0) continue;
            const uint32_t incl = snk_wave_scan_incl(nb);
            lf = w_frags + (uint32_t)__popcll(hm & ((1ull << tid) - 1ull));
            rel = w_bases + incl - nb;
            w_frags += (uint32_t)__popcll(hm);
            w_bases += (uint32_t)__builtin_amdgcn_readlane((int)incl, 63);
        } else if (head) {
            lf = atomicAdd(&fcnt, 1u);
            rel = atomicAdd(&bcnt, nb);
        }
        if (head) describe(lf, rel, fwd ? tL : tR, fwd ? tR : tL, cnt, i, !fwd, GR ? (uint32_t)own_key(q, i).lo : 0u);
    }
    for (uint32_t i = tid; i < n; i += T) {
        if (w_next(2 * i) == FM) continue;
        uint32_t cur = i << 1, cnt = 1;
        const snk_kmer ki = key_of(i);
        bool closed = false;
        while (cnt <= n) {
            const uint32_t l = lnk[cur];
            if (l == NONE16) break;
            const uint32_t j = l >> 1;
            if (j == i) { closed = true; break; }
            if (snk_kmer_lt(key_of(j), ki)) break;
            cur = l ^ 1u;
            ++cnt;
        }
        if (closed) {
            const unsigned long long xf = atomicAdd(&xp.cur[0], 1ull);
            const unsigned long long xb = atomicAdd(&xp.cur[1], (unsigned long long)(cnt + K - 1));
            if (xf < xp.fcap && xb + cnt + K - 1 <= xp.bcap) {
                uint32_t e = i << 1;
                for (uint32_t q = 1; q < cnt; ++q) e = lnk[e] ^ 1u;
                const uint64_t f = xp.f0 + xf, bo = xp.b0 + xb;
                const uint32_t pid = (i << 1) | 1u;
                nk[f] = cnt;
                hl_self[2 * f] = 2ull * ((DIST ? da.my_node_off : 0ull) + ch.base) + pid;
                hl_self[2 * f + 1] = 2ull * ((DIST ? da.my_node_off : 0ull) + ch.base) + e;
                hl_nb[2 * f] = NONE64;
                hl_nb[2 * f + 1] = NONE64;
                bstart[f] = bo;
                if (sfrag) { sfrag[2 * ch.base + pid] = (uint32_t)(2 * f); sfrag[2 * ch.base + e] = (uint32_t)(2 * f + 1); }
                if (GR) fgroup[f] = (uint32_t)ki.lo;
                snk_kmer k = ki;
                for (int b = 0; b < K; ++b) fbases[bo + b] = (uint8_t)oriented_base<K>(k, false, b);
                uint32_t curs = i << 1;
                for (uint32_t pos = 1; pos < cnt; ++pos) {
                    const uint32_t l = lnk[curs];
                    k = key_of(l >> 1);
                    fbases[bo + (K - 1) + pos] = (uint8_t)oriented_base<K>(k, (l & 1u) == 0, K - 1);
                    curs = l ^ 1u;
                }
            }
        }
    }
    __syncthreads();
#pragma unroll
    for (int q = 0; q < NPT; ++q) {
        const uint32_t i = tid + q * T;
        if (i >= n || w_next(2 * i) != FM) continue;
        const uint32_t tR = w_tail(2 * i), tL = w_tail(2 * i + 1), dR = w_dist(2 * i), dL = w_dist(2 * i + 1);
        const bool fwd = tL < tR;
        const uint32_t pos = fwd ? dL : dR;
        if (pos == 0) continue;
        const snk_kmer k = own_key(q, i);
        uint32_t fo = foffL[fwd ? tL : tR];
        if constexpr (WIDE) fo = frel[fo];
        fbases[c_boff + fo + (K - 1) + pos] = (uint8_t)oriented_base<K>(k, !fwd, K - 1);
    }
    struct __attribute__((packed)) u32_any { uint32_t v; };
    uint32_t nheads = w_frags;
    if constexpr (!ONEW) nheads = fcnt;
    constexpr int HPI = T / 16;
    static_assert(K % 4 == 0 && K / 4 <= 16, "a head is K / 4 dwords, one per lane of its group");
    for (uint32_t h0 = 0; h0 < nheads; h0 += HPI) {
        const uint32_t h = h0 + (tid >> 4);
        const int q = tid & 15;
        const bool act = h < nheads && q < K / 4;
        const uint32_t hn = act ? hnode[h] : 0u;
        const uint32_t i = hn >> 1;
        const bool rc = hn & 1u;
        snk_kmer k;
        if constexpr (ONEW) {
            k.hi = 0; k.lo = 0;
#pragma unroll
            for (int s = 0; s < NPT; ++s) {
                if ((uint32_t)(s * T) >= n) break;
                const int src = (int)(i & 63u);
                const uint32_t a0 = (uint32_t)__shfl((int)(uint32_t)(kq[s].hi >> 32), src), a1 = (uint32_t)__shfl((int)(uint32_t)kq[s].hi, src);
                const uint32_t a2 = (uint32_t)__shfl((int)(uint32_t)(kq[s].lo >> 32), src);
                uint32_t a3 = 0;
                if constexpr (K > 48) a3 = (uint32_t)__shfl((int)(uint32_t)kq[s].lo, src);
                if ((i >> 6) == (uint32_t)s) { k.hi = ((uint64_t)a0 << 32) | a1; k.lo = ((uint64_t)a2 << 32) | a3; }
            }
        } else {
            k = key_of(i);
        }
        if (act) {
            uint32_t fo;
            if constexpr (WIDE) fo = frel[h];
            else { const uint32_t tR = w_tail(2 * i), tL = w_tail(2 * i + 1); fo = foffL[tL < tR ? tL : tR]; }
            const uint32_t v = oriented_base<K>(k, rc, 4 * q) | (oriented_base<K>(k, rc, 4 * q + 1) << 8) | (oriented_base<K>(k, rc, 4 * q + 2) << 16) |
                               (oriented_base<K>(k, rc, 4 * q + 3) << 24);
            reinterpret_cast<u32_any*>(fbases + c_boff + fo + 4 * q)->v = v;
        }
    }
}

__global__ void __launch_bounds__(TB) bl_chunk_bases_kernel(const uint4* __restrict__ desc, const uint32_t* __restrict__ nfrag, uint32_t nchunks,
                                                            uint32_t K, uint64_t* __restrict__ nbases) {
    const uint32_t c = blockIdx.x * TB + threadIdx.x;
    if (c > nchunks) return;
    if (c == nchunks) { nbases[c] = 0; return; }
    const uint32_t n = desc[c].y;
    nbases[c] = nfrag[c] ? (uint64_t)n + (uint64_t)(K - 1) * nfrag[c] : 0ull;
}

__global__ void __launch_bounds__(TB) bl_pack_vals_kernel(const uint32_t* __restrict__ counts, const uint8_t* __restrict__ ctx,
                                                          uint64_t n, uint64_t* __restrict__ vals) {
    const uint64_t i = (uint64_t)blockIdx.x * TB + threadIdx.x;
    if (i < n) vals[i] = ((uint64_t)counts[i] << 8) | ctx[i];
}
__global__ void __launch_bounds__(TB) bl_unpack_vals_kernel(const uint64_t* __restrict__ vals, uint64_t n,
                                                            uint32_t* __restrict__ counts, uint8_t* __restrict__ ctx) {
    const uint64_t i = (uint64_t)blockIdx.x * TB + threadIdx.x;
    if (i < n) { counts[i] = (uint32_t)(vals[i] >> 8); ctx[i] = (uint8_t)(vals[i] & 0xFFu); }
}

}

constexpr int SCAP = 256, ST = 64;
constexpr int BCAP = SNK_GRAPH_CHUNK_MAX, BT = 256;

namespace {
constexpr int QWORDS = 4;
constexpr int QSPAN = 8 * QWORDS * TB;
template <int K, bool FILL>
__global__ void __launch_bounds__(TB) bl_query_kernel(const snk_u128* __restrict__ keys, const uint8_t* __restrict__ premote, uint64_t n,
                                                      uint32_t NB_total, uint32_t NBl, uint32_t world, uint32_t mlen,
                                                      unsigned long long* __restrict__ qcount_or_cursor,
                                                      unsigned long long* __restrict__ qbuf) {
    extern __shared__ unsigned long long dynq[];
    __shared__ uint16_t list[QSPAN];
    __shared__ uint32_t cnt;
    uint32_t* lcur = reinterpret_cast<uint32_t*>(dynq + world);
    const uint64_t base = (uint64_t)blockIdx.x * QSPAN;
    if (threadIdx.x == 0) cnt = 0;
    for (uint32_t r = threadIdx.x; r < world; r += TB) { dynq[r] = 0; lcur[r] = 0; }
    __syncthreads();
    for (int t = 0; t < QWORDS; ++t) {
        const uint32_t w0 = 8u * ((uint32_t)t * TB + threadIdx.x);
        const uint64_t i8 = base + w0;
        unsigned long long w = 0;
        if (i8 + 8 <= n) w = *reinterpret_cast<const unsigned long long*>(premote + i8);
        else for (uint64_t q = i8; q < n; ++q) w |= (unsigned long long)premote[q] << (8 * (q - i8));
        if (w) {
            uint32_t m = 0;
            for (int q = 0; q < 8; ++q) if ((w >> (8 * q)) & 0xFFull) ++m;
            uint32_t pos = atomicAdd(&cnt, m);
            for (int q = 0; q < 8; ++q) if ((w >> (8 * q)) & 0xFFull) list[pos++] = (uint16_t)(w0 + q);
        }
    }
    __syncthreads();
    const uint32_t m = cnt;
    for (uint32_t it = threadIdx.x; it < m; it += TB) {
        const uint64_t i = base + list[it];
        const snk_kmer k = load_key(keys, i);
        for (uint32_t rem = premote[i]; rem; rem &= rem - 1) {
            const uint32_t bit = __ffs(rem) - 1;
            const snk_kmer y = bit < 4 ? snk_kmer_succ<K>(k, bit) : snk_kmer_pred<K>(k, bit - 4);
            const uint32_t owner = (mlen == (uint32_t)SNK_M_LONG ? snk_bucket_of_kmer<K, SNK_M_LONG>(y, NB_total) : snk_bucket_of_kmer<K, SNK_M_OF(K)>(y, NB_total)) / NBl;
            atomicAdd(&dynq[owner], 1ull);
        }
    }
    __syncthreads();
    for (uint32_t r = threadIdx.x; r < world; r += TB) {
        const unsigned long long c = dynq[r];
        if (c) dynq[r] = FILL ? atomicAdd(&qcount_or_cursor[r], c) : (atomicAdd(&qcount_or_cursor[r], c), 0ull);
    }
    if (!FILL) return;
    __syncthreads();
    for (uint32_t it = threadIdx.x; it < m; it += TB) {
        const uint64_t i = base + list[it];
        const snk_kmer k = load_key(keys, i);
        for (uint32_t rem = premote[i]; rem; rem &= rem - 1) {
            const uint32_t bit = __ffs(rem) - 1;
            const snk_kmer y = bit < 4 ? snk_kmer_succ<K>(k, bit) : snk_kmer_pred<K>(k, bit - 4);
            const uint32_t owner = (mlen == (uint32_t)SNK_M_LONG ? snk_bucket_of_kmer<K, SNK_M_LONG>(y, NB_total) : snk_bucket_of_kmer<K, SNK_M_OF(K)>(y, NB_total)) / NBl;
            const snk_kmer r = snk_kmer_rc<K>(y);
            const bool rev = snk_kmer_lt(r, y);
            const snk_kmer c = rev ? r : y;
            const unsigned long long slot = dynq[owner] + atomicAdd(&lcur[owner], 1u);
            qbuf[3 * slot + 0] = c.lo;
            qbuf[3 * slot + 1] = c.hi;
            qbuf[3 * slot + 2] = (unsigned long long)i | ((unsigned long long)bit << 32) | ((unsigned long long)(rev ? 1 : 0) << 40);
        }
    }
}
}

template <int K, bool GR>
static int bl_prune_impl(snk_ctx* ctx, hipStream_t st, snk_bl_state* B, char* err, size_t errcap) {
    const snk_table* tab = B->tab;
    const uint64_t n = tab->n;
    chunk_src cs;
    cs.chunk_n = tab->chunk_n;
    cs.chunk_base = tab->chunk_base;
    cs.extra = tab->extra;
    cs.region_off = tab->region_off;
    cs.NB = tab->NB;
    cs.n_extra = tab->n_extra;
    cs.n_regions = tab->n_regions;
    cs.span = nullptr;
    const uint32_t merge_cap = snk_opt_is_set(ctx, SNK_OPT_chunk_merge) ? std::min<uint32_t>(snk_opt_u32(ctx, SNK_OPT_chunk_merge), (uint32_t)SCAP) : (uint32_t)SCAP;
    if (merge_cap && tab->chunk_n && tab->NB > tab->n_regions) {
        uint8_t* span;
        uint32_t* merged;
        G_ALLOC(span, uint8_t, (uint64_t)tab->NB + 1);
        G_ALLOC(merged, uint32_t, (uint64_t)tab->NB + 1);
        SNK_HIP_TRY(snk_launch(bl_chunk_merge_kernel, snk_blocks(tab->n_regions, 256), 256, 0, st, tab->chunk_n, tab->chunk_base, tab->NB, tab->n_regions, merge_cap, span, merged));
        cs.span = span;
        cs.chunk_n = merged;
    }
    const uint32_t nchunks = tab->NB + tab->n_extra;
    B->nchunks = nchunks;
    G_ALLOC(B->desc, uint4, (uint64_t)nchunks + 1);
    uint64_t* desc_src = nullptr;
    if (tab->keys_r) G_ALLOC(desc_src, uint64_t, (uint64_t)nchunks + 1);
    SNK_HIP_TRY(snk_launch(bl_chunk_desc_kernel, snk_blocks(nchunks, 256), 256, 0, st, cs, nchunks, B->desc, tab->region_cap, desc_src));
    uint32_t *nbnd, *ctr;
    G_ALLOC(B->ctx, uint8_t, n + 16);
    G_ALLOC(B->pend, uint8_t, n + 16);
    G_ALLOC(B->counts, uint32_t, n + 4);
    G_ALLOC(B->nbr, uint32_t, n + 2);
    G_ALLOC(B->rq, uint32_t, 2 * n + 2);
    G_ALLOC(nbnd, uint32_t, (uint64_t)nchunks + 1);
    G_ALLOC(B->biglist, uint32_t, n / SCAP + 2);
    G_ALLOC(ctr, uint32_t, 16);
    B->premote = nullptr;
    if (B->world > 1 || B->force_dist) {
        G_ALLOC(B->premote, uint8_t, n + 16);
        SNK_HIP_TRY(hipMemsetAsync(B->premote, 0, n + 16, st));
    }
    SNK_HIP_TRY(hipMemsetAsync(nbnd, 0, ((uint64_t)nchunks + 1) * 4, st));
    SNK_HIP_TRY(hipMemsetAsync(ctr, 0, 64, st));
    bl_shard sh;
    sh.bucket_base = B->premote ? B->rank * B->NBl : 0u;
    sh.NBl = B->premote ? B->NBl : 0u;
    sh.me = B->rank;
    sh.G = tab->n_regions ? tab->n_regions : 1u;
    sh.premote = B->premote;
    const uint32_t NBh = B->premote ? B->NB_total : tab->NB;
    const uint32_t cpw = snk_opt_u32(ctx, SNK_OPT_bl_cpw);
    uint64_t tg0 = 0;
    unsigned long long* index0 = nullptr;
    if (snk_opt_u32(ctx, SNK_OPT_bl_index_fused)) {
        const uint64_t guess = (ctx->last_bnd_n == n && ctx->last_bnd) ? ctx->last_bnd + ctx->last_bnd / 8 : n / 5;
        tg0 = 1024;
        while (tg0 < 2 * guess) tg0 <<= 1;
        G_ALLOC(index0, unsigned long long, tg0 + 1);
        SNK_HIP_TRY(hipMemsetAsync(index0, 0, (tg0 + 1) * 8, st));
    }
    unsigned long long* spec = nullptr;
    if (B->want_spec) {
        G_ALLOC(spec, unsigned long long, BL_SPEC_WORDS);
        SNK_HIP_TRY(hipMemsetAsync(spec, 0, (size_t)BL_SPEC_WORDS * 8, st));
    }
    bl_regions rg;
    rg.keys_r = tab->keys_r; rg.vals_r = tab->vals_r; rg.desc_src = desc_src;
    rg.keys_dense = const_cast<snk_u128*>(tab->keys);
    const bool long_m = ctx->mlen == (uint32_t)SNK_M_LONG;
    SNK_HIP_TRY(snk_launch(long_m ? bl_prune_kernel<K, SCAP, ST, false, GR, SNK_M_LONG> : bl_prune_kernel<K, SCAP, ST, false, GR, SNK_M_OF(K)>, snk_blocks(nchunks, cpw), ST, 0, st, (const uint4*)B->desc, NBh, sh, rg,
                           (const uint32_t*)nullptr, nchunks, cpw, tab->keys, tab->vals, B->do_prune | (snk_opt_u32(ctx, SNK_OPT_bl_noclassify) ? 2u : 0u), B->ctx, B->counts, B->pend, B->nbr, nbnd,
                           B->biglist, ctr, (const uint32_t*)nullptr, index0, tg0 - 1, spec));
    uint32_t h_nbig = 0;
    SNK_HIP_TRY(hipMemcpyAsync(ctr + 1, ctr, 4, hipMemcpyDeviceToDevice, st));
    SNK_HIP_TRY(snk_launch(long_m ? bl_prune_kernel<K, BCAP, BT, true, GR, SNK_M_LONG> : bl_prune_kernel<K, BCAP, BT, true, GR, SNK_M_OF(K)>, 2048, BT, 0, st, (const uint4*)B->desc, NBh, sh, rg,
                           (const uint32_t*)B->biglist, 0u, 1u, tab->keys, tab->vals, B->do_prune | (snk_opt_u32(ctx, SNK_OPT_bl_noclassify) ? 2u : 0u), B->ctx, B->counts, B->pend, B->nbr,
                           nbnd, B->biglist, ctr + 2, (const uint32_t*)(ctr + 1), index0, tg0 - 1, spec));
    if (spec) SNK_HIP_TRY(snk_launch(bl_spec_fold_kernel, 1, BL_SPEC_LDS, 0, st, spec));
    if (tab->keys_r) {
        snk_ctx_release_block(ctx, tab->keys_r);
        snk_ctx_release_block(ctx, tab->vals_r);
    }
    unsigned long long* d_sum;
    G_ALLOC(d_sum, unsigned long long, 2);
    {
        size_t tb = 0;
        auto in = rocprim::make_transform_iterator(nbnd, [] __device__(uint32_t v) { return (unsigned long long)v; });
        SNK_HIP_TRY(rocprim::reduce((void*)nullptr, tb, in, d_sum, 0ull, (size_t)nchunks, rocprim::plus<unsigned long long>(), st));
        void* tmp;
        int rc = snk_ctx_alloc(ctx, tb, &tmp, err, errcap);
        if (rc) return rc;
        SNK_HIP_TRY(rocprim::reduce(tmp, tb, in, d_sum, 0ull, (size_t)nchunks, rocprim::plus<unsigned long long>(), st));
    }
    unsigned long long h_bnd = 0, h_gaveup = 0, h_spec_over = 0;
    if (index0) SNK_HIP_TRY(hipMemcpyAsync(&h_gaveup, index0 + tg0, 8, hipMemcpyDeviceToHost, st));
    if (spec) SNK_HIP_TRY(hipMemcpyAsync(&h_spec_over, spec + BL_SPEC_OVER, 8, hipMemcpyDeviceToHost, st));
    SNK_HIP_TRY(hipMemcpyAsync(&h_bnd, d_sum, 8, hipMemcpyDeviceToHost, st));
    SNK_HIP_TRY(hipMemcpyAsync(&h_nbig, ctr + 1, 4, hipMemcpyDeviceToHost, st));
    SNK_HIP_TRY(snk_sync(st));
    B->nbig = h_nbig;
    B->spec = spec;
    B->spec_over = h_spec_over != 0;
    B->n_boundary = h_bnd;
    ctx->last_bnd = h_bnd; ctx->last_bnd_n = n;
    uint64_t tg = 1024;
    while (tg < 2 * h_bnd) tg <<= 1;
    const bool fused_ok = index0 && !h_gaveup && h_bnd * 4 <= tg0 * 3;
    if (fused_ok) { B->index = index0; tg = tg0; }
    else {
        if (index0) snk_ctx_release_block(ctx, index0);
        G_ALLOC(B->index, unsigned long long, tg);
        SNK_HIP_TRY(hipMemsetAsync(B->index, 0, tg * 8, st));
    }
    B->index_mask = tg - 1;
    if (h_bnd) {
        if (!fused_ok) SNK_HIP_TRY(snk_launch(bl_index_build_kernel, snk_blocks(n, TB), TB, 0, st, tab->keys, B->pend, n, B->index, tg - 1));
        SNK_HIP_TRY(snk_launch(bl_resolve_kernel<K, GR>, snk_blocks(n, 8 * TB), TB, 0, st, tab->keys, B->pend, n,
                               B->index, tg - 1, B->do_prune, B->ctx, B->rq, (const uint8_t*)B->premote));
    }
    return SNK_OK;
}

template <int K, bool DIST, bool GR>
static int bl_fragments_impl(snk_ctx* ctx, hipStream_t st, snk_bl_state* B, const bl_dist_args& da, snk_frag_out* out, char* err,
                             size_t errcap) {
    const snk_table* tab = B->tab;
    const uint32_t nchunks = B->nchunks, h_nbig = B->nbig;
    uint32_t *nfrag, *foff;
    uint64_t *nbases, *boff;
    G_ALLOC(nfrag, uint32_t, (uint64_t)nchunks + 1);
    G_ALLOC(foff, uint32_t, (uint64_t)nchunks + 1);
    G_ALLOC(nbases, uint64_t, (uint64_t)nchunks + 1);
    G_ALLOC(boff, uint64_t, (uint64_t)nchunks + 1);
    SNK_HIP_TRY(hipMemsetAsync(nfrag, 0, ((uint64_t)nchunks + 1) * 4, st));
    bl_extra_pool xp0;
    memset(&xp0, 0, sizeof xp0);
    SNK_HIP_TRY(snk_launch(bl_frag_kernel<K, SCAP, ST, false, false, DIST, GR>, nchunks, ST, 0, st, (const uint4*)B->desc,
                           (const uint32_t*)nullptr, tab->keys, B->ctx, B->pend, B->nbr, B->rq, da, nfrag, (const uint32_t*)nullptr,
                           (const uint64_t*)nullptr, (uint32_t*)nullptr, (unsigned long long*)nullptr, (unsigned long long*)nullptr,
                           (uint64_t*)nullptr, (uint8_t*)nullptr, (uint32_t*)nullptr, (uint32_t*)nullptr, xp0));
    SNK_HIP_TRY(snk_launch(bl_frag_kernel<K, BCAP, BT, true, false, DIST, GR>, h_nbig, BT, 0, st, (const uint4*)B->desc,
                           (const uint32_t*)B->biglist, tab->keys, B->ctx, B->pend, B->nbr, B->rq, da, nfrag, (const uint32_t*)nullptr,
                           (const uint64_t*)nullptr, (uint32_t*)nullptr, (unsigned long long*)nullptr, (unsigned long long*)nullptr,
                           (uint64_t*)nullptr, (uint8_t*)nullptr, (uint32_t*)nullptr, (uint32_t*)nullptr, xp0));
    SNK_HIP_TRY(snk_launch(bl_chunk_bases_kernel, snk_blocks((uint64_t)nchunks + 1, TB), TB, 0, st, (const uint4*)B->desc, nfrag, nchunks,
                           (uint32_t)K, nbases));
    int rc;
    if ((rc = excl_scan<uint32_t>(ctx, st, nfrag, foff, (size_t)nchunks + 1, err, errcap))) return rc;
    if ((rc = excl_scan<uint64_t>(ctx, st, nbases, boff, (size_t)nchunks + 1, err, errcap))) return rc;
    uint32_t h_F = 0;
    uint64_t h_B = 0;
    SNK_HIP_TRY(hipMemcpyAsync(&h_F, foff + nchunks, 4, hipMemcpyDeviceToHost, st));
    SNK_HIP_TRY(hipMemcpyAsync(&h_B, boff + nchunks, 8, hipMemcpyDeviceToHost, st));
    SNK_HIP_TRY(snk_sync(st));
    unsigned long long* xcur;
    G_ALLOC(xcur, unsigned long long, 2);
    const uint32_t pool0 = snk_opt_u32(ctx, SNK_OPT_bl_pool);
    uint64_t xf_cap = pool0 ? pool0 + h_F / 256 : 0, xb_cap = xf_cap * (K + 63);
    unsigned long long h_x[2] = {0, 0};
    for (int attempt = 0; attempt < 2; ++attempt) {
        ctx->last_bl_attempts = (uint32_t)attempt + 1;
        G_ALLOC(out->nk, uint32_t, (uint64_t)h_F + xf_cap + 1);
        G_ALLOC(out->hl_self, unsigned long long, 2ull * (h_F + xf_cap) + 2);
        G_ALLOC(out->hl_nb, unsigned long long, 2ull * (h_F + xf_cap) + 2);
        G_ALLOC(out->boff, uint64_t, (uint64_t)h_F + xf_cap + 2);
        G_ALLOC(out->bases, uint8_t, h_B + xb_cap + 16);
        out->fgroup = nullptr;
        if (GR) G_ALLOC(out->fgroup, uint32_t, (uint64_t)h_F + xf_cap + 1);
        G_ALLOC(out->sfrag, uint32_t, 2 * tab->n + 2);
        SNK_HIP_TRY(hipMemsetAsync(xcur, 0, 16, st));
        bl_extra_pool xp;
        xp.cur = xcur;
        xp.f0 = h_F;
        xp.b0 = h_B;
        xp.fcap = xf_cap;
        xp.bcap = xb_cap;
        SNK_HIP_TRY(snk_launch(bl_frag_kernel<K, SCAP, ST, false, true, DIST, GR>, nchunks, ST, 0, st, (const uint4*)B->desc,
                               (const uint32_t*)nullptr, tab->keys, B->ctx, B->pend, B->nbr, B->rq, da, nfrag, foff, boff, out->nk, out->hl_self,
                               out->hl_nb, out->boff, out->bases, out->fgroup, out->sfrag, xp));
        SNK_HIP_TRY(snk_launch(bl_frag_kernel<K, BCAP, BT, true, true, DIST, GR>, h_nbig, BT, 0, st, (const uint4*)B->desc,
                               (const uint32_t*)B->biglist, tab->keys, B->ctx, B->pend, B->nbr, B->rq, da, nfrag, foff, boff, out->nk,
                               out->hl_self, out->hl_nb, out->boff, out->bases, out->fgroup, out->sfrag, xp));
        SNK_HIP_TRY(hipMemcpyAsync(h_x, xcur, 16, hipMemcpyDeviceToHost, st));
        SNK_HIP_TRY(snk_sync(st));
        if (h_x[0] <= xf_cap && h_x[1] <= xb_cap) break;
        if (attempt == 1) return snk_fail(SNK_E_INTERNAL, err, errcap, "bucket-local graph: circle pool overflow");
        xf_cap = h_x[0] + 64;
        xb_cap = h_x[1] + 64;
    }
    out->n_frags = h_F + h_x[0];
    out->total_bases = h_B + h_x[1];
    out->n_local_circles = (uint32_t)h_x[0];
    ctx->last_bl_circles = h_x[0];
    ctx->last_bl_big_chunks = h_nbig;
    return SNK_OK;
}

template <int K, bool GR>
static int local_graph_impl(snk_ctx* ctx, hipStream_t st, const snk_table* tab, uint32_t do_prune, bool want_unitigs,
                            bool sort_table, snk_graph_out* out, snk_u128** keys_final, float* ms, char* err, size_t errcap) {
    memset(out, 0, sizeof *out);
    const uint64_t n = tab->n;
    *keys_final = tab->keys;
    if (n == 0) {
        int rc0 = snk_spectrum(ctx, st, nullptr, 0, &out->spectrum, &out->spectrum_bins, err, errcap);
        if (rc0) return rc0;
        G_ALLOC(out->unitig_off, uint64_t, 2);
        SNK_HIP_TRY(hipMemsetAsync(out->unitig_off, 0, 16, st));
        G_ALLOC(out->unitig_bases, uint8_t, 16);
        G_ALLOC(out->ctx, uint8_t, 16);
        G_ALLOC(out->counts, uint32_t, 4);
        return SNK_OK;
    }
    if (n >= (1ull << 31)) return snk_fail(SNK_E_UNSUPPORTED, err, errcap, "more than 2^31 retained k-mers on one GPU (%llu)", (unsigned long long)n);
#ifndef SNK_DBG_NO_CHUNK_CHECK
    if (snk_count_slots(K) > (uint32_t)BCAP + 768u + 64u)
#else
    if (false)
#endif
        return snk_fail(SNK_E_INTERNAL, err, errcap, "bucket-local graph: chunk capacity %d is below the count table's limit", BCAP);
    snk_phase_timer tm(st);
    tm.mark();
    snk_bl_state B;
    memset(&B, 0, sizeof B);
    B.tab = tab;
    B.K = K;
    B.world = 1;
    B.do_prune = do_prune;
    B.want_spec = sort_table ? 0u : 1u;
    int rc = bl_prune_impl<K, GR>(ctx, st, &B, err, errcap);
    if (rc) return rc;
    tm.mark();
    tm.mark();
    out->n_boundary = B.n_boundary;
    if (want_unitigs) {
        snk_frag_out fo;
        memset(&fo, 0, sizeof fo);
        bl_dist_args da;
        memset(&da, 0, sizeof da);
        if ((rc = bl_fragments_impl<K, false, GR>(ctx, st, &B, da, &fo, err, errcap))) return rc;
        tm.mark();
        snk_join_out jo;
        rc = snk_dist_join(ctx, st, K, fo.n_frags, fo.nk, fo.hl_self, fo.hl_nb, fo.boff, fo.bases, fo.total_bases, &jo, err, errcap, fo.fgroup, fo.sfrag, 2 * n);
        if (rc) return rc;
        tm.mark();
        out->n_unitigs = jo.n_unitigs;
        out->total_bases = jo.total_bases;
        out->unitig_off = jo.unitig_off;
        out->unitig_bases = jo.unitig_bases;
        out->unitig_group = jo.unitig_group;
        out->n_circles = jo.n_circles;
        out->rank_rounds = jo.rank_rounds;
        out->n_fragments = fo.n_frags;
    } else {
        G_ALLOC(out->unitig_off, uint64_t, 2);
        SNK_HIP_TRY(hipMemsetAsync(out->unitig_off, 0, 16, st));
        G_ALLOC(out->unitig_bases, uint8_t, 16);
        tm.mark();
        tm.mark();
    }
    out->ctx = B.ctx;
    out->counts = B.counts;
    if (sort_table) {
        uint64_t *v_in, *v_out;
        snk_u128* k_out;
        G_ALLOC(v_in, uint64_t, n + 1);
        G_ALLOC(v_out, uint64_t, n + 1);
        G_ALLOC(k_out, snk_u128, n + 1);
        SNK_HIP_TRY(snk_launch(bl_pack_vals_kernel, snk_blocks(n, TB), TB, 0, st, B.counts, B.ctx, n, v_in));
        rc = snk_graph_sort(ctx, st, K, n, tab->keys, v_in, k_out, v_out, err, errcap);
        if (rc) return rc;
        SNK_HIP_TRY(snk_launch(bl_unpack_vals_kernel, snk_blocks(n, TB), TB, 0, st, v_out, n, B.counts, B.ctx));
        *keys_final = k_out;
    }
    if (B.spec && !B.spec_over) {
        out->spectrum = B.spec;
        out->spectrum_bins = BL_SPEC_BINS;
    } else if ((rc = snk_spectrum(ctx, st, B.counts, n, &out->spectrum, &out->spectrum_bins, err, errcap))) return rc;
    tm.mark();
    if (ms) { ms[0] = tm.ms(0, 1); ms[1] = tm.ms(1, 2); ms[2] = tm.ms(2, 3); ms[3] = tm.ms(3, 4); ms[4] = tm.ms(4, 5); }
    return SNK_OK;
}

int snk_local_graph(snk_ctx* ctx, hipStream_t st, uint32_t K, const snk_table* tab, uint32_t do_prune, bool want_unitigs,
                    bool sort_table, bool grouped, snk_graph_out* out, snk_u128** keys_final, float* ms, char* err, size_t errcap) {
    if (tab->sorted) return snk_fail(SNK_E_INTERNAL, err, errcap, "bucket-local graph needs the table in chunk order");
    if (grouped) {
        if (K != 48) return snk_fail(SNK_E_UNSUPPORTED, err, errcap, "grouped graphs need K=48");
        return local_graph_impl<48, true>(ctx, st, tab, do_prune, want_unitigs, sort_table, out, keys_final, ms, err, errcap);
    }
    if (K == 48) return local_graph_impl<48, false>(ctx, st, tab, do_prune, want_unitigs, sort_table, out, keys_final, ms, err, errcap);
    if (K == 60) return local_graph_impl<60, false>(ctx, st, tab, do_prune, want_unitigs, sort_table, out, keys_final, ms, err, errcap);
    return snk_fail(SNK_E_UNSUPPORTED, err, errcap, "K=%u is not supported (48 or 60)", K);
}

int snk_bl_dist_plan(snk_ctx* ctx, hipStream_t st, snk_bl_state* B, char* err, size_t errcap) {
    B->force_dist = 1;
    const uint64_t n = B->tab->n;
    G_ALLOC(B->qcount, unsigned long long, B->world + 4);
    G_ALLOC(B->qcursor, unsigned long long, B->world + 1);
    G_ALLOC(B->rq_idx, uint32_t, 2 * n + 2);
    G_ALLOC(B->rq_meta, uint16_t, 2 * n + 2);
    SNK_HIP_TRY(hipMemsetAsync(B->qcount, 0, (B->world + 1) * 8ull, st));
    SNK_HIP_TRY(hipMemsetAsync(B->rq_idx, 0xFF, (2 * n + 2) * 4, st));
    if (n == 0) {
        G_ALLOC(B->ctx, uint8_t, 16);
        G_ALLOC(B->counts, uint32_t, 4);
        G_ALLOC(B->index, unsigned long long, 1024);
        SNK_HIP_TRY(hipMemsetAsync(B->index, 0, 1024 * 8, st));
        B->index_mask = 1023;
        return SNK_OK;
    }
    if (n >= (1ull << 31)) return snk_fail(SNK_E_UNSUPPORTED, err, errcap, "more than 2^31 retained k-mers on one GPU (%llu)", (unsigned long long)n);
    int rc = B->K == 48 ? bl_prune_impl<48, false>(ctx, st, B, err, errcap) : bl_prune_impl<60, false>(ctx, st, B, err, errcap);
    if (rc) return rc;
    const size_t lds = (size_t)B->world * 12 + 16;
    const uint64_t grid = snk_blocks(n, QSPAN);
    if (B->K == 48) SNK_HIP_TRY(snk_launch(bl_query_kernel<48, false>, grid, TB, lds, st, B->tab->keys, (const uint8_t*)B->premote, n, B->NB_total, B->NBl, B->world, ctx->mlen, B->qcount, (unsigned long long*)nullptr));
    else SNK_HIP_TRY(snk_launch(bl_query_kernel<60, false>, grid, TB, lds, st, B->tab->keys, (const uint8_t*)B->premote, n, B->NB_total, B->NBl, B->world, ctx->mlen, B->qcount, (unsigned long long*)nullptr));
    return SNK_OK;
}
int snk_bl_dist_fill(snk_ctx* ctx, hipStream_t st, snk_bl_state* B, const unsigned long long* d_qoff, void* d_qbuf, char* err, size_t errcap) {
    const uint64_t n = B->tab->n;
    if (n == 0) return SNK_OK;
    SNK_HIP_TRY(hipMemcpyAsync(B->qcursor, d_qoff, (B->world + 1) * 8ull, hipMemcpyDeviceToDevice, st));
    const size_t lds = (size_t)B->world * 12 + 16;
    const uint64_t grid = snk_blocks(n, QSPAN);
    if (B->K == 48) SNK_HIP_TRY(snk_launch(bl_query_kernel<48, true>, grid, TB, lds, st, B->tab->keys, (const uint8_t*)B->premote, n, B->NB_total, B->NBl, B->world, ctx->mlen, B->qcursor, (unsigned long long*)d_qbuf));
    else SNK_HIP_TRY(snk_launch(bl_query_kernel<60, true>, grid, TB, lds, st, B->tab->keys, (const uint8_t*)B->premote, n, B->NB_total, B->NBl, B->world, ctx->mlen, B->qcursor, (unsigned long long*)d_qbuf));
    return SNK_OK;
}
int snk_bl_dist_fragments(snk_ctx* ctx, hipStream_t st, snk_bl_state* B, const unsigned long long* d_node_off, unsigned long long my_node_off,
                          snk_frag_out* out, char* err, size_t errcap) {
    memset(out, 0, sizeof *out);
    const uint64_t n = B->tab->n;
    {
        int rc0 = snk_spectrum(ctx, st, n ? B->counts : nullptr, n, &out->spectrum, &out->spectrum_bins, err, errcap);
        if (rc0) return rc0;
    }
    if (n == 0) {
        G_ALLOC(out->boff, uint64_t, 2);
        SNK_HIP_TRY(hipMemsetAsync(out->boff, 0, 16, st));
        G_ALLOC(out->bases, uint8_t, 16);
        G_ALLOC(out->nk, uint32_t, 4);
        G_ALLOC(out->hl_self, unsigned long long, 2);
        G_ALLOC(out->hl_nb, unsigned long long, 2);
        return SNK_OK;
// ... 10 lines not shown
```

### supernova_amd/csrc/snk_pipeline.hip

```cpp
#include <string.h>
#include <cstring>
#include <rocprim/rocprim.hpp>

#include <stdlib.h>
#include <math.h>

#include <algorithm>
#include <vector>

#include "snk_ctx.h"
#include "snk_common.h"
#include "snk_graph.h"
#include "snk_kernels.h"
#include "snk_stages.h"

namespace {

__global__ void widen_offsets_kernel(const uint32_t* __restrict__ in, uint64_t* __restrict__ out, uint32_t n) {
    uint32_t i = blockIdx.x * blockDim.x + threadIdx.x;
    if (i < n) out[i] = in[i];
}

__global__ void __launch_bounds__(256) input_fp_kernel(const uint4* __restrict__ rows16, uint64_t n16, const uint4* __restrict__ aux16, uint64_t m16,
                                                       unsigned long long* __restrict__ out) {
    unsigned long long acc = 0;
    for (int s = 0; s < 16; ++s) {
        const uint64_t q = (uint64_t)(threadIdx.x * 16 + s);
        if (n16) {
            const uint64_t at = (n16 / 4096) * q + (q * 0x9E37u) % (n16 / 4096 + 1);
            if (at < n16) { const uint4 v = rows16[at]; acc += snk_mix64(((unsigned long long)v.x << 32 | v.y) ^ snk_mix64(((unsigned long long)v.z << 32 | v.w) + at)); }
        }
        if (m16) {
            const uint64_t at = (m16 / 4096) * q + (q * 0x79B9u) % (m16 / 4096 + 1);
            if (at < m16) { const uint4 v = aux16[at]; acc += snk_mix64(((unsigned long long)v.x << 32 | v.y) ^ snk_mix64(((unsigned long long)v.z << 32 | v.w) + at + 0x51ED27ull)); }
        }
    }
    for (int off = 32; off > 0; off >>= 1) acc += __shfl_xor(acc, off);
    if ((threadIdx.x & 63) == 0) atomicAdd(out, acc);
}

typedef snk_phase_timer phase_timer;


}

static int graph_tail(snk_ctx* ctx, hipStream_t st, const snk_params* p, uint32_t K, bool grouped, bool local_graph, uint64_t n_reads, unsigned long long h_ninst,
                      snk_table& tab, const snk_partition& part, snk_dev_result* out, phase_timer& tm, char* err, size_t errcap) {
    int rc;
    void* records = part.records;
    if (h_ninst) {
        snk_sizing_history& H = ctx->sizing;
        H.store(snk_sizing_key(K, grouped, ctx->mlen), n_reads, (ctx->count_screen && !grouped && H.screen_ratio > 0.0) ? H.screen_ratio : (double)tab.distinct / (double)h_ninst,
                (double)tab.n / (double)h_ninst);
    }
    snk_ctx_release_block(ctx, records);
    const uint64_t n_kmers = tab.n;
    out->buckets_split = tab.buckets_split;
    out->max_slots_used = tab.max_slots_used;
    out->n_kmers = n_kmers;
    out->keys = tab.keys;
    tm.mark();
    tm.mark();

    snk_graph_out go;
    ctx->last_bl_attempts = ctx->last_bl_big_chunks = 0;
    ctx->last_bl_circles = 0;
    if (local_graph) {
        snk_u128* keys_final = nullptr;
        rc = snk_local_graph(ctx, st, K, &tab, p->min_freq > 1 ? 1u : 0u, !(p->flags & SNK_F_NO_GRAPH),
                             !(p->flags & SNK_F_UNSORTED_TABLE), grouped, &go, &keys_final, out->graph_ms, err, errcap);
        if (rc) return rc;
        out->keys = keys_final;
        out->n_boundary = go.n_boundary;
        out->n_fragments = go.n_fragments;
    } else {
        rc = snk_graph_build(ctx, st, K, tab.keys, tab.vals, n_kmers, p->min_freq > 1 ? 1u : 0u, !(p->flags & SNK_F_NO_GRAPH), &go,
                             err, errcap);
        if (rc) return rc;
    }
    tm.mark();
    SNK_HIP_TRY(snk_sync(st));
    out->counts = go.counts;
    out->ctx = go.ctx;
    out->spectrum = go.spectrum;
    out->spectrum_bins = go.spectrum_bins;
    out->n_unitigs = go.n_unitigs;
    out->unitig_total_bases = go.total_bases;
    out->unitig_off = go.unitig_off;
    out->unitig_bases = go.unitig_bases;
    out->unitig_group = go.unitig_group;
    out->n_circles = go.n_circles;
    out->rank_rounds = go.rank_rounds;
    out->phase_ms[0] = tm.ms(0, 1);
    out->phase_ms[1] = tm.ms(1, 2);
    out->phase_ms[2] = tm.ms(2, 3);
    out->phase_ms[3] = tab.count_ms;
    out->phase_ms[4] = tab.sort_ms;
    out->phase_ms[5] = tm.ms(5, 6);
    out->phase_ms[7] = tm.ms(0, 6);
    out->kernel_ms[0] = 0.f;
    out->kernel_ms[1] = part.kernel_ms;
    out->kernel_ms[2] = tab.count_kernel_ms;
    out->scratch_bytes = ctx->peak_alloc;
    return SNK_OK;
}

namespace {

struct count_call {
    snk_ctx* ctx; hipStream_t st; const snk_dev_reads* in; const snk_params* p; snk_dev_result* out;
    bool grouped, local_graph, fused;
    const uint16_t* good_len;
    snk_fused_trim ft;
    uint32_t* status;
    unsigned long long ub_inst, ub_live;
    phase_timer* tm;
    char* err; size_t errcap;
    uint32_t NB;
    bool first, want_pilot;
    uint64_t ovf_floor;
    snk_partition part; snk_table tab;
    unsigned long long h_ninst;
    double retarget_ratio;
    uint64_t ovf_want;
};

snk_count_job count_job_of(const count_call& C, const void* records, const uint64_t* seg, uint32_t nseg, unsigned long long n_inst, snk_count_pilot* pilot) {
    snk_count_job cj;
    cj.K = C.p->K; cj.records = records; cj.seg_beg = seg; cj.seg_end = seg + C.NB; cj.seg_stride = 2 * C.NB; cj.nseg = nseg; cj.NB = C.NB;
    cj.min_freq = C.p->min_freq; cj.bc_mode = (C.in->bc && !C.grouped) ? C.p->min_bc : 0u; cj.grouped = C.grouped ? 1u : 0u;
    cj.n_inst_hint = n_inst; cj.status = C.status; cj.want_sort = !C.local_graph; cj.defer_compact = C.local_graph;
    cj.pilot = C.want_pilot ? pilot : nullptr;
    return cj;
}

#ifdef SNK_PROBES
struct overlap_probe {
    uint32_t mode = 0;
    hipStream_t s2 = nullptr, s2hi = nullptr, sp2 = nullptr;
    hipEvent_t pe[3] = {nullptr, nullptr, nullptr};
    ~overlap_probe() {
        for (auto& e : pe) if (e) (void)hipEventDestroy(e);
        if (s2) (void)hipStreamDestroy(s2);
        if (s2hi) (void)hipStreamDestroy(s2hi);
    }
    int start(snk_ctx* ctx, hipStream_t st, char* err, size_t errcap) {
        mode = snk_opt_u32(ctx, SNK_OPT_overlap_probe);
        if (!mode) return SNK_OK;
        { SNK_HIP_TRY(hipStreamCreateWithFlags(&s2, hipStreamNonBlocking)); int lo = 0, hi = 0; (void)hipDeviceGetStreamPriorityRange(&lo, &hi); SNK_HIP_TRY(hipStreamCreateWithPriority(&s2hi, hipStreamNonBlocking, hi)); }
        sp2 = (mode & 4u) ? s2hi : s2;
        for (auto& e : pe) SNK_HIP_TRY(hipEventCreate(&e));
        SNK_HIP_TRY(hipEventRecord(pe[0], st));
        SNK_HIP_TRY(hipStreamWaitEvent(sp2, pe[0], 0));
        SNK_HIP_TRY(hipEventRecord(pe[1], sp2));
        int rc = snk_probe_relaunch_msp(ctx, sp2, snk_opt_u32(ctx, SNK_OPT_overlap_probe_dbg), err, errcap);
        if (rc) return rc;
        SNK_HIP_TRY(hipEventRecord(pe[2], sp2));
        if ((mode & 3u) == 2u) SNK_HIP_TRY(hipStreamSynchronize(sp2));
        return SNK_OK;
    }
    int report(const snk_partition& part, const snk_table& tab, char* err, size_t errcap) {
        if (!mode) return SNK_OK;
        SNK_HIP_TRY(hipStreamSynchronize(sp2));
        float pm = 0.f;
        (void)hipEventElapsedTime(&pm, pe[1], pe[2]);
        fprintf(stderr, "[snk overlap probe] mode %u: partition kernel (first launch, alone) %.2f ms; relaunched %s %.2f ms; count kernel %.2f ms; count stage %.2f ms\n", mode,
                part.kernel_ms, (mode & 3u) == 2u ? "alone" : "next to the count kernel", pm, tab.count_kernel_ms, tab.count_ms);
        return SNK_OK;
    }
};
#endif

int count_in_passes(count_call& C, uint32_t n_passes) {
    snk_ctx* ctx = C.ctx;
    snk_dev_result* out = C.out;
    const uint32_t NB = C.NB;
    int rc;
    snk_partition_passes PS;
    if ((rc = snk_partition_passes_open(ctx, C.st, C.p->K, C.in, C.good_len, C.fused ? &C.ft : nullptr, NB, n_passes, C.ub_inst, C.ub_live, C.grouped, &PS, C.err, C.errcap, C.ovf_floor))) return rc;
    if (C.first) C.tm->mark();
    std::vector<snk_hot> pass_hots;
    PS.hots = &pass_hots;
    snk_count_ranges rgs{n_passes, PS.bounds, snk_partition_passes_run, &PS, true, &pass_hots};
    rgs.finished = [](void* u) {
        snk_partition_passes* S = static_cast<snk_partition_passes*>(u);
        snk_ctx_release_block(S->ctx, S->records); S->records = nullptr;
        snk_ctx_release_block(S->ctx, S->ovf_bucket); S->ovf_bucket = nullptr;
    };
    snk_count_pilot pilot{0.0, nullptr, nullptr};
    snk_count_job cj = count_job_of(C, PS.records, PS.seg, 2u, C.ub_inst, &pilot);
    cj.ranges = &rgs;
    rc = snk_stage_count_table(ctx, C.st, cj, &C.tab, C.err, C.errcap);
    if (rc == SNK_OVF_RETRY) C.ovf_want = PS.ovf_want;
    if (rc == SNK_RETARGET) {
        const unsigned long long inst_now = PS.h_plan[0] ? PS.h_plan[0] : C.ub_inst;
        C.retarget_ratio = inst_now ? pilot.per_bucket * (double)NB / (double)inst_now : 0.0;
    }
    if (rc) return rc;
    C.h_ninst = PS.h_plan[0];
    snk_partition& part = C.part;
    memset(&part, 0, sizeof part);
    part.NB = NB; part.cap = PS.cap; part.nseg = 2; part.n_overflow = (uint32_t)std::min<uint64_t>(PS.n_overflow, 0xFFFFFFFFull); part.n_supermers = PS.n_supermers;
    part.records = PS.records; part.cursor = PS.cursor; part.seg = PS.seg; part.kernel_ms = PS.kernel_ms;
    out->n_instances = C.h_ninst;
    out->n_supermers = part.n_supermers;
    out->n_overflow = part.n_overflow;
    out->n_hot_buckets = PS.n_hot;
    return SNK_OK;
}

int count_in_one_pass(count_call& C) {
    snk_ctx* ctx = C.ctx;
    snk_dev_result* out = C.out;
    snk_partition& part = C.part;
    unsigned long long h_plan[2] = {C.ub_inst, C.ub_live};
    int rc = snk_stage_partition(ctx, C.st, C.p->K, C.in, C.good_len, C.NB, h_plan[0], h_plan[1], C.grouped, C.status, &part, C.err, C.errcap, nullptr, C.fused ? h_plan : nullptr,
                                 C.fused ? &C.ft : nullptr, true);
    if (rc) return rc;
    C.h_ninst = h_plan[0];
// ... 272 lines not shown
```

### supernova_amd/lib.py

```python
from __future__ import annotations

import ctypes as C
from pathlib import Path

import os as _os

_HERE = Path(__file__).resolve().parent
LIB_PATH = Path(_os.environ.get("SNK_LIB_PATH", str(_HERE / "libsnk.so")))


class SnkError(RuntimeError):
    def __init__(self, code: int, msg: str):
        super().__init__(f"libsnk error {code}: {msg}")
        self.code = code


class SnkParams(C.Structure):
    _fields_ = [("K", C.c_uint32), ("min_qual", C.c_uint32), ("min_freq", C.c_uint32), ("min_bc", C.c_uint32),
                ("n_buckets", C.c_uint32), ("flags", C.c_uint32)]


class SnkSynthParams(C.Structure):
    _fields_ = [("seed", C.c_uint64), ("n_reads", C.c_uint64), ("genome_len", C.c_uint64), ("read_len", C.c_uint32),
                ("mol_len", C.c_uint32), ("mols_per_bc", C.c_uint32), ("pairs_per_bc", C.c_uint32),
# ... 215 lines not shown

    def to_dict(self) -> dict:
        none = (1 << 64) - 1
        d = {f: int(getattr(self, f)) for f in ("levels", "n_kmers", "n_unitigs", "n_circles", "n_palindromes", "n_bases", "n_instances",
                                                "table_digest", "unitig_digest", "peak_bytes")}
        d["counters"] = {n: int(self.count[i]) for i, n in enumerate(CHECK_COUNTERS)}
        d["first"] = {n: int(self.first[i]) for i, n in enumerate(CHECK_COUNTERS) if int(self.first[i]) != none}
        d["violations"] = sum(d["counters"].values())
        d["graph_ms"], d["reads_ms"] = float(self.graph_ms), float(self.reads_ms)
        return d


RANK_WYLLIE, RANK_RULING, RANK_RULING_THEN_WYLLIE = 1, 2, 3


class SnkRankEvidence(C.Structure):
    _fields_ = [("n_circles", C.c_uint32), ("rounds", C.c_uint32), ("source", C.c_uint32), ("ruling_attempts", C.c_uint32), ("splitters", C.c_uint64),
                ("sparse_cut", C.c_uint32), ("bad", C.c_uint32), ("part_attempts", C.c_uint32), ("partitioned", C.c_uint32), ("reserved", C.c_uint64 * 4)]

    def to_dict(self) -> dict:
        return {f: int(getattr(self, f)) for f, _ in self._fields_ if f != "reserved"}


COMM_A2A = C.CFUNCTYPE(C.c_int, C.c_void_p, C.c_void_p, C.POINTER(C.c_uint64), C.POINTER(C.c_uint64), C.c_void_p, C.POINTER(C.c_uint64),
                       C.POINTER(C.c_uint64), C.c_uint32)
COMM_GATHER = C.CFUNCTYPE(C.c_int, C.c_void_p, C.c_void_p, C.c_uint32, C.POINTER(C.c_uint64), C.c_uint32)
RANGE_READY = C.CFUNCTYPE(C.c_int, C.c_void_p, C.c_uint32)

_lib = None


def load() -> C.CDLL:
    global _lib
    if _lib is not None:
        return _lib
    if not LIB_PATH.exists():
        raise FileNotFoundError(
            f"{LIB_PATH} is missing: run `python -m supernova_amd.build` (hipcc, gfx950). "
            "supernova_amd has no CPU fallback.")
    _preload_hip_runtime()
    lib = C.CDLL(str(LIB_PATH))
    _declare(lib)
    _lib = lib
    return lib


def _preload_hip_runtime() -> None:
    import os
    cands = []
    try:
        import torch
        cands.append(Path(torch.__file__).parent / "lib" / "libamdhip64.so")
    except Exception:
        pass
    cands += [Path(os.environ.get("ROCM_PATH", "/opt/rocm")) / "lib" / "libamdhip64.so"]
    for c in cands:
        if c.exists():
            C.CDLL(str(c), mode=C.RTLD_GLOBAL)
            return
    raise FileNotFoundError("no libamdhip64.so found (torch bundle or $ROCM_PATH/lib)")


def _declare(lib: C.CDLL) -> None:
    vp, u32, u64, i32 = C.c_void_p, C.c_uint32, C.c_uint64, C.c_int32
    cp, sz = C.c_char_p, C.c_size_t
    P = C.POINTER
    sig = {
        "snk_version": (cp, []),
        "snk_last_error": (cp, []),
        "snk_params_default": (None, [P(SnkParams)]),
        "snk_ctx_create": (C.c_int, [C.c_int, P(vp), cp, sz]),
        "snk_ctx_destroy": (None, [vp]),
        "snk_ctx_trim": (None, [vp]),
        "snk_ctx_reserve": (C.c_int, [vp, u64, cp, sz]),
        "snk_tuning_default": (None, [P(SnkTuning)]),
        "snk_ctx_set_tuning": (C.c_int, [vp, P(SnkTuning), cp, sz]),
        "snk_ctx_get_tuning": (None, [vp, P(SnkTuning)]),
        "snk_ctx_set_option": (C.c_int, [vp, cp, C.c_longlong, cp, sz]),
        "snk_option_check": (C.c_int, [cp, C.c_longlong, cp, sz]),
        "snk_ctx_clear_option": (C.c_int, [vp, cp]),
        "snk_ctx_get_option": (C.c_int, [vp, cp, P(C.c_longlong)]),
        "snk_option_name": (cp, [u32]),
        "snk_option_doc": (cp, [u32]),
        "snk_synth_default": (None, [P(SnkSynthParams), u64, u64, C.c_int]),
        "snk_synth_set_errors": (None, [P(SnkSynthParams), u32]),
        "snk_synth_host": (C.c_int, [P(SnkSynthParams), u64, u64, vp, u32, vp, u32, vp]),
        "snk_synth_dev": (C.c_int, [vp, P(SnkSynthParams), u64, u64, vp, u32, vp, u32, vp, vp]),
        "snk_dev_trim": (C.c_int, [vp, vp, u32, vp, u32, u64, u32, u32, vp, vp]),
        "snk_dev_pack_ascii": (C.c_int, [vp, vp, u32, u32, u64, vp, u32, vp]),
        "snk_dev_count_graph": (C.c_int, [vp, P(SnkDevReads), P(SnkParams), P(SnkDevResult), vp, cp, sz]),
        "snk_dev_stream_begin": (C.c_int, [vp, P(SnkParams), u32, u64, C.c_int, vp, cp, sz]),
        "snk_dev_stream_append": (C.c_int, [vp, P(SnkDevReads), vp, cp, sz]),
        "snk_dev_stream_finish": (C.c_int, [vp, P(SnkDevResult), vp, cp, sz]),
        "snk_dev_download": (C.c_int, [vp, vp, vp, sz, vp]),
        "snk_count_graph": (C.c_int, [vp, P(SnkReads), P(SnkParams), P(SnkResult), cp, sz]),
        "snk_free": (None, [P(SnkResult)]),
        "snk_host_alloc_pinned": (C.c_int, [sz, P(vp), cp, sz]),
        "snk_host_free_pinned": (None, [vp]),
        "snk_write_bv": (C.c_int, [cp, u64, vp, vp, cp, sz]),
        "snk_read_bv": (C.c_int, [cp, P(u64), P(P(u64)), P(P(C.c_uint8)), cp, sz]),
        "snk_hbv_from_unitigs": (C.c_int, [u32, u64, vp, vp, P(SnkHbv), cp, sz]),
        "snk_dev_hbv": (C.c_int, [vp, u32, u64, vp, vp, P(SnkHbv), P(C.c_float), vp, cp, sz]),
        "snk_dev_bv_image": (C.c_int, [vp, u32, u64, vp, vp, C.c_int, P(C.c_void_p), P(u64), vp, cp, sz]),
        "snk_hbv_free": (None, [P(SnkHbv)]),
        "snk_dev_path_reads": (C.c_int, [vp, u32, P(SnkDevReads), u64, vp, vp, P(SnkHbv), P(SnkDevPaths), vp, cp, sz]),
        "snk_dev_path_reads2": (C.c_int, [vp, u32, P(SnkDevReads), u64, vp, vp, P(SnkHbv), u32, P(SnkDevPaths), vp, cp, sz]),
        "snk_dev_mark_dups": (C.c_int, [vp, P(SnkDevReads), P(SnkDevPaths), P(SnkDevDups), vp, cp, sz]),
        "snk_dev_paths_index": (C.c_int, [vp, P(SnkDevPaths), u64, vp, P(SnkDevPidx), vp, cp, sz]),
        "snk_dev_edge_barcodes": (C.c_int, [vp, P(SnkDevPaths), vp, u64, vp, u32, P(SnkDevEbcx), vp, cp, sz]),
        "snk_write_ebcx": (C.c_int, [cp, u64, vp, vp, cp, sz]),
        "snk_read_ebcx": (C.c_int, [cp, P(u64), P(P(u64)), P(P(i32)), cp, sz]),
        "snk_dev_paths_zip": (C.c_int, [vp, P(SnkDevPaths), P(SnkHbv), P(SnkDevPathsx), vp, cp, sz]),
        "snk_dev_paths_unzip": (C.c_int, [vp, P(SnkDevPathsx), P(SnkHbv), P(SnkDevPaths), vp, cp, sz]),
        "snk_dev_extend_paths": (C.c_int, [vp, u32, P(SnkDevReads), u64, vp, vp, P(SnkHbv), P(SnkDevPaths), u32, P(SnkDevExtend), vp, cp, sz]),
        "snk_dev_mark_bads": (C.c_int, [vp, u32, P(SnkDevReads), u64, vp, vp, P(SnkHbv), P(SnkDevPaths), u32, P(SnkDevBads), vp, cp, sz]),
        "snk_dev_edge_pairs": (C.c_int, [vp, u32, u64, vp, vp, P(SnkHbv), vp, P(SnkDevPaths), P(SnkDevPidx), vp, vp, u32, u32, P(SnkDevHops), vp, cp, sz]),
        "snk_write_hops": (C.c_int, [cp, u64, vp, cp, sz]),
        "snk_dev_close_gaps": (C.c_int, [vp, u32, u64, vp, vp, P(SnkHbv), vp, P(SnkDevReads), P(SnkDevPaths), P(SnkDevPidx), u64, vp, u32, u32, u32, P(SnkDevClosures),
                                        vp, cp, sz]),
        "snk_read_hops": (C.c_int, [cp, P(u64), P(P(i32)), cp, sz]),
        "snk_dev_mark_bads_df": (C.c_int, [vp, u32, vp, u64, u64, u32, u32, u64, u64, vp, vp, P(SnkHbv), P(SnkDevPaths), u32, P(SnkDevBads), cp, sz]),
        "snk_patch_plan_sizes": (C.c_int, [u32, u64, vp, P(SnkHbv), u64, vp, P(SnkPatchPlan), cp, sz]),
        "snk_dev_patch_pieces": (C.c_int, [vp, u32, u64, vp, vp, P(SnkHbv), u64, vp, vp, u64, vp, vp, u64, vp, P(SnkDevPieces), vp, cp, sz]),
        "snk_dev_patch_merge": (C.c_int, [vp, u32, P(SnkDevResult), vp, u64, P(SnkDevPatchUnitigs), vp, cp, sz]),
        "snk_dev_patch_paths": (C.c_int, [vp, u32, u64, vp, vp, P(SnkHbv), u64, vp, vp, P(SnkHbv), P(SnkDevPaths), P(SnkDevPatched), vp, cp, sz]),
        "snk_dev_delete_edges": (C.c_int, [vp, u32, u64, vp, vp, P(SnkHbv), vp, P(SnkDevPaths), vp, u64, u32, P(SnkDevEdit), vp, cp, sz]),
        "snk_dev_edit_free": (None, [P(SnkDevEdit)]),
        "snk_dev_hanging_ends": (C.c_int, [vp, u32, u64, vp, vp, P(SnkHbv), vp, P(SnkDevPaths), u32, u32, P(SnkDevHanging), vp, cp, sz]),
        "snk_write_pathsx": (C.c_int, [cp, u64, vp, u64, vp, u64, cp, sz]),
        "snk_read_pathsx": (C.c_int, [cp, P(u64), P(u64), P(P(C.c_int64)), P(u64), P(P(C.c_uint8)), cp, sz]),
        "snk_write_hbx": (C.c_int, [cp, u32, u64, vp, vp, P(SnkHbv), cp, sz]),
        "snk_write_paths": (C.c_int, [cp, u64, vp, vp, vp, vp, cp, sz]),
        "snk_write_paths_index": (C.c_int, [cp, cp, u64, vp, vp, vp, cp, sz]),
        "snk_write_dup": (C.c_int, [cp, u64, vp, cp, sz]),
        "snk_hbv_involution": (C.c_int, [P(SnkHbv), u64, vp, cp, sz]),
        "snk_write_hbv": (C.c_int, [cp, cp, u32, u64, vp, vp, P(SnkHbv), cp, sz]),
        "snk_read_fastb": (C.c_int, [cp, P(u64), P(u32), P(P(C.c_uint16)), P(P(u32)), cp, sz]),
        "snk_read_qualp": (C.c_int, [cp, u64, u32, vp, cp, sz]),
        "snk_read_bci": (C.c_int, [cp, u64, vp, P(u64), cp, sz]),
        "snk_read_fasth": (C.c_int, [cp, u32, P(u64), P(u32), P(P(C.c_uint8)), P(P(C.c_uint8)), P(P(C.c_uint16)), P(P(C.c_uint8)), cp, sz]),
        "snk_host_free": (None, [vp]),
        "snk_bc_index_create": (C.c_int, [vp, cp, sz, P(vp), cp, sz]),
        "snk_bc_index_destroy": (None, [vp]),
        "snk_bc_index_lines": (u32, [vp]),
        "snk_dev_bc_ids": (C.c_int, [vp, vp, vp, u32, u64, vp, vp, cp, sz]),
        "snk_pack2_bytes": (u64, [u64]),
        "snk_dev_pack2": (C.c_int, [vp, vp, u64, vp, vp]),
        "snk_dev_unpack2": (C.c_int, [vp, vp, u64, vp, vp]),
        "snk_host_cpu_budget": (u32, []),
        "snk_ctx_last_partition_passes": (u32, [vp]),
        "snk_ctx_last_count_limit": (u32, [vp]),
        "snk_ctx_last_hbv_flood": (u32, [vp, P(u64), P(u64)]),
        "snk_ctx_last_local_graph": (u32, [vp, P(u64), P(u32)]),
        "snk_fasth_open": (C.c_int, [P(cp), u32, u32, u32, u32, u32, P(vp), cp, sz]),
        "snk_fasth_next": (C.c_int, [vp, P(SnkFasthBatch), cp, sz]),
        "snk_fasth_release": (None, [vp, P(SnkFasthBatch)]),
        "snk_fasth_file_pairs": (u64, [vp, u32]),
        "snk_fasth_close": (None, [vp]),
        "snk_dev_ingest_fasth": (C.c_int, [vp, P(cp), u32, u32, vp, u32, u32, P(SnkDevIngest), cp, sz]),
        "snk_dev_ingest_free": (None, [P(SnkDevIngest)]),
        "snk_dev_ingest_count_graph": (C.c_int, [vp, P(cp), u32, u32, vp, u32, u32, u64, P(SnkParams), P(SnkDevResult), P(SnkDevIngest), cp, sz]),
        "snk_df_open": (C.c_int, [cp, cp, cp, P(vp), P(SnkDfInfo), cp, sz]),
        "snk_df_close": (None, [vp]),
        "snk_df_max_len": (C.c_int, [vp, vp, u64, u64, P(u32), cp, sz]),
        "snk_dev_ingest_df": (C.c_int, [vp, vp, u64, u64, u32, u32, u64, P(SnkDevIngest), cp, sz]),
        "snk_dev_ingest_df_trimmed": (C.c_int, [vp, vp, u64, u64, u32, u32, u64, u32, u32, P(SnkDevIngest), cp, sz]),
        "snk_dev_ingest_df_count_graph": (C.c_int, [vp, vp, u64, u64, u32, u32, u64, P(SnkParams), C.c_int64, P(SnkDevResult), P(SnkDevIngest), cp, sz]),
        "snk_write_df": (C.c_int, [cp, u64, vp, u32, vp, u32, vp, u32, vp, u32, u64, cp, sz]),
        "snk_synth_df_write": (C.c_int, [cp, P(SnkSynthParams), u64, u64, u32, u32, cp, sz]),
        "snk_synth_fasth_write": (C.c_int, [cp, P(SnkSynthParams), u64, u64, C.c_int, P(u64), cp, sz]),
        "snk_synth_bc_seq": (None, [u32, vp]),
        "snk_comm_set_rccl_path": (C.c_int, [cp]),
        "snk_comm_unique_id": (C.c_int, [vp, cp, sz]),
        "snk_comm_create_rccl": (C.c_int, [vp, vp, u32, u32, P(vp), cp, sz]),
        "snk_comm_from_nccl": (C.c_int, [vp, vp, u32, u32, P(vp), cp, sz]),
        "snk_comm_create_local": (C.c_int, [u32, P(vp), cp, sz]),
        "snk_comm_create_callbacks": (C.c_int, [u32, u32, COMM_A2A, COMM_GATHER, vp, P(vp), cp, sz]),
        "snk_comm_selftest": (C.c_int, [vp, u64, u32, u32, cp, sz]),
        "snk_comm_destroy": (None, [vp]),
        "snk_comm_abort": (None, [vp]),
        "snk_comm_rank": (u32, [vp]),
        "snk_comm_world": (u32, [vp]),
        "snk_comm_kind": (cp, [vp]),
        "snk_shard_step": (C.c_int, [vp, vp, P(SnkDevReads), P(SnkParams), u64, u32, P(SnkShardResult), vp, cp, sz]),
        "snk_shard_stream_begin": (C.c_int, [vp, vp, P(SnkParams), u32, u64, u64, C.c_int, vp, cp, sz]),
        "snk_shard_stream_append": (C.c_int, [vp, P(SnkDevReads), vp, cp, sz]),
        "snk_shard_stream_finish": (C.c_int, [vp, vp, u32, P(SnkShardResult), vp, cp, sz]),
        "snk_shard_gather_unitigs": (C.c_int, [vp, vp, P(SnkShardResult), u32, u32, u32, P(SnkResult), vp, cp, sz]),
        "snk_dev_check_graph": (C.c_int, [vp, P(SnkCheckInput), P(SnkDevReads), P(SnkCheckReport), vp, cp, sz]),
        "snk_dev_rank_lists": (C.c_int, [vp, u64, vp, vp, vp, u32, P(u64), vp, P(SnkRankEvidence), vp, cp, sz]),
    }
    for name, (res, args) in sig.items():
        fn = getattr(lib, name)
        fn.restype = res
        fn.argtypes = args
    lib._snk_declared = tuple(sig)


ERRCAP = 512


def call(fn, *args) -> None:
    err = C.create_string_buffer(ERRCAP)
    rc = fn(*args, err, ERRCAP)
    if rc:
        raise SnkError(rc, err.value.decode(errors="replace"))


def check(code: int) -> None:
    if code != 0:
        raise SnkError(code, load().snk_last_error().decode(errors="replace"))


def exported_symbols() -> tuple[str, ...]:
    return load()._snk_declared
```

Measured before the change: 102.3.

## Add mid-size chunk class with 512-capacity prune and fragment kernels

Chunks are now sorted into small, mid (257-512) and big classes when their descriptors are built, using wave ballots and one atomic per block to fill the mid and big lists. Mid chunks no longer fall through to the 256-thread full-capacity kernels. They go to 64-thread, 512-capacity prune and fragment kernels with smaller shared-memory tables and 32-bit ranking records. This is meant to cut the LDS and occupancy cost of handling moderately oversized chunks. The trade-off is an extra kernel launch per phase, more template instantiations, and a changed bit layout for the hop-count field in the ranking records.

Measured after the change: 102.9, median of 4. No clear change (+0.6%).

```diff
diff --git a/include/snk.h b/include/snk.h
--- a/include/snk.h
+++ b/include/snk.h
@@ -282,6 +282,7 @@
                          snk_hbv* out, char* err, size_t errcap);
 uint32_t snk_ctx_last_hbv_flood(const snk_ctx* ctx, uint64_t* device_components, uint64_t* host_components);
 uint32_t snk_ctx_last_local_graph(const snk_ctx* ctx, uint64_t* in_chunk_circles, uint32_t* big_chunks);
+void snk_ctx_last_chunk_classes(const snk_ctx* ctx, uint32_t classes[3]);
 int snk_dev_hbv(snk_ctx* ctx, uint32_t K, uint64_t n_unitigs, const void* d_unitig_off, const void* d_unitig_bases,
                 snk_hbv* out, float* device_ms, void* stream, char* err, size_t errcap);
 void snk_hbv_free(snk_hbv* h);
diff --git a/supernova_amd/csrc/snk_api.hip b/supernova_amd/csrc/snk_api.hip
--- a/supernova_amd/csrc/snk_api.hip
+++ b/supernova_amd/csrc/snk_api.hip
@@ -383,6 +383,10 @@
     if (big_chunks) *big_chunks = ctx ? ctx->last_bl_big_chunks : 0u;
     return ctx ? ctx->last_bl_attempts : 0u;
 }
+extern "C" void snk_ctx_last_chunk_classes(const snk_ctx* ctx, uint32_t classes[3]) {
+    if (!classes) return;
+    for (int j = 0; j < 3; ++j) classes[j] = ctx ? ctx->last_bl_classes[j] : 0u;
+}
 extern "C" uint32_t snk_ctx_last_count_limit(const snk_ctx* ctx) { return ctx ? ctx->last_count_limit : 0u; }
 extern "C" int snk_ctx_reserve(snk_ctx* ctx, uint64_t bytes, char* err, size_t errcap) {
     if (!ctx) return snk_fail(SNK_E_ARG, err, errcap, "snk_ctx_reserve: NULL context");
diff --git a/supernova_amd/csrc/snk_ctx.h b/supernova_amd/csrc/snk_ctx.h
--- a/supernova_amd/csrc/snk_ctx.h
+++ b/supernova_amd/csrc/snk_ctx.h
@@ -62,6 +62,7 @@
     uint64_t last_hbv_dev_components = 0, last_hbv_host_components = 0;
     uint32_t last_bl_attempts = 0, last_bl_big_chunks = 0;
     uint64_t last_bl_circles = 0;
+    uint32_t last_bl_classes[3] = {0, 0, 0};
     std::vector<unsigned long long> h_region_off;
     snk_opts opts;
     void* shard = nullptr;
diff --git a/supernova_amd/csrc/snk_dist.hip b/supernova_amd/csrc/snk_dist.hip
--- a/supernova_amd/csrc/snk_dist.hip
+++ b/supernova_amd/csrc/snk_dist.hip
@@ -19,6 +19,7 @@
     S->rank = rank; S->world = world; S->NB_total = NB_total; S->NBl = NB_total / world;
     S->circ_all = nullptr; S->join_circles = 0;
     ctx->last_bl_attempts = ctx->last_bl_big_chunks = 0; ctx->last_bl_circles = 0;
+    ctx->last_bl_classes[0] = ctx->last_bl_classes[1] = ctx->last_bl_classes[2] = 0;
     return S;
 }
 
diff --git a/supernova_amd/csrc/snk_graph.h b/supernova_amd/csrc/snk_graph.h
--- a/supernova_amd/csrc/snk_graph.h
+++ b/supernova_amd/csrc/snk_graph.h
@@ -112,8 +112,8 @@
     const snk_table* tab;
     uint32_t K, rank, world, NB_total, NBl, do_prune, force_dist;
     uint4* desc;
-    uint32_t nchunks, nbig;
-    uint32_t* biglist;
+    uint32_t nchunks, nmid, nbig;
+    uint32_t *midlist, *biglist;
     uint8_t *ctx, *pend, *premote;
     uint32_t *counts, *nbr, *rq;
     uint32_t* rq_idx;
diff --git a/supernova_amd/csrc/snk_local.hip b/supernova_amd/csrc/snk_local.hip
--- a/supernova_amd/csrc/snk_local.hip
+++ b/supernova_amd/csrc/snk_local.hip
@@ -9,6 +9,10 @@
 #include "snk_kernels.h"
 #include "snk_graph.h"
 #include "snk_stages.h"
+
+constexpr int SCAP = 256, ST = 64;
+constexpr int MCAP = 512, MT = 64;
+constexpr int BCAP = SNK_GRAPH_CHUNK_MAX, BT = 256;
 
 namespace {
 
@@ -59,11 +63,15 @@
         expect = base + n;
     }
 }
-__global__ void __launch_bounds__(256) bl_chunk_desc_kernel(chunk_src cs, uint32_t nchunks, uint4* __restrict__ desc, uint64_t region_cap, uint64_t* __restrict__ desc_src) {
-    const uint32_t c = blockIdx.x * 256 + threadIdx.x;
-    if (c >= nchunks) return;
-    uint32_t bucket, n, off = 0, meta = 0, region;
-    if (c < cs.NB) {
+constexpr int DESC_T = 1024;
+__global__ void __launch_bounds__(DESC_T) bl_chunk_desc_kernel(chunk_src cs, uint32_t nchunks, uint4* __restrict__ desc, uint64_t region_cap, uint64_t* __restrict__ desc_src,
+                                                            uint32_t* __restrict__ midlist, uint32_t* __restrict__ biglist, uint32_t* __restrict__ ctr) {
+    __shared__ uint32_t wsum[2][DESC_T / 64 + 1];
+    const uint32_t c = blockIdx.x * DESC_T + threadIdx.x;
+    const bool live = c < nchunks;
+    uint32_t bucket = 0, n = 0, off = 0, meta = 0, region = 0;
+    if (!live) {
+    } else if (c < cs.NB) {
         bucket = c; n = cs.chunk_n[c];
         if (n) off = cs.chunk_base[c];
         region = bucket % cs.n_regions;
@@ -72,9 +80,26 @@
         const uint4 e = cs.extra[c - cs.NB];
         bucket = e.x; off = e.y; n = e.z & 0xFFFu; region = e.z >> 12; meta = e.w;
     }
-    const uint64_t base = cs.region_off[region] + off;
-    desc[c] = make_uint4((uint32_t)base, n, bucket, meta);
-    if (desc_src) desc_src[c] = (uint64_t)region * region_cap + off;
+    if (live) {
+        const uint64_t base = cs.region_off[region] + off;
+        desc[c] = make_uint4((uint32_t)base, n, bucket, meta);
+        if (desc_src) desc_src[c] = (uint64_t)region * region_cap + off;
+    }
+    const bool on[2] = {n > (uint32_t)SCAP && n <= (uint32_t)MCAP, n > (uint32_t)MCAP};
+    const uint32_t lane = threadIdx.x & 63u, wave = threadIdx.x >> 6;
+    const unsigned long long m[2] = {__ballot(on[0]), __ballot(on[1])};
+    if (lane < 2) wsum[lane][wave] = (uint32_t)__popcll(m[lane]);
+    __syncthreads();
+    if (threadIdx.x < 2) {
+        uint32_t total = 0;
+        for (int w = 0; w < DESC_T / 64; ++w) { const uint32_t v = wsum[threadIdx.x][w]; wsum[threadIdx.x][w] = total; total += v; }
+        wsum[threadIdx.x][DESC_T / 64] = total ? atomicAdd(&ctr[threadIdx.x], total) : 0u;
+    }
+    __syncthreads();
+    uint32_t* const list[2] = {midlist, biglist};
+#pragma unroll
+    for (int l = 0; l < 2; ++l)
+        if (on[l]) list[l][wsum[l][DESC_T / 64] + wsum[l][wave] + (uint32_t)__popcll(m[l] & ((1ull << lane) - 1ull))] = c;
 }
 __device__ __forceinline__ chunk_t chunk_get(const uint4* __restrict__ desc, uint32_t c) {
     const uint4 d = desc[c];
@@ -112,19 +137,18 @@
     for (int r = 0; r < BL_SPEC_REPL; ++r) s += rep[r * BL_SPEC_LDS + threadIdx.x];
     spec[threadIdx.x] += s;
 }
-template <int K, int CAP, int T, bool BIG, bool GR, int MM>
+template <int K, int CAP, int T, bool GR, int MM>
 __device__ __forceinline__ void bl_prune_chunk(const uint32_t c, const uint4* __restrict__ desc, uint32_t NB, bl_shard sh, const bl_regions& rg,
                                                      const snk_u128* __restrict__ keys, const uint64_t* __restrict__ vals,
                                                      uint32_t do_prune, uint8_t* __restrict__ ctx_out,
                                                      uint32_t* __restrict__ count_out, uint8_t* __restrict__ pend_out,
                                                      uint32_t* __restrict__ nbr_out, uint32_t* __restrict__ nbnd,
-                                                     uint32_t* __restrict__ biglist, uint32_t* __restrict__ nbig,
                                                      unsigned long long* __restrict__ gindex, uint64_t gmask,
                                                      unsigned long long* __restrict__ spec, uint32_t* __restrict__ shist) {
-    constexpr int HT = CAP <= 256 ? 512 : 4096;
+    constexpr int HT = CAP <= 256 ? 512 : CAP <= 512 ? 1024 : 4096;
     typedef typename std::conditional<(K <= 48 && !GR), uint32_t, uint64_t>::type klo_w;
     constexpr int KLS = (K <= 48 && !GR) ? 32 : 0;
-    constexpr bool ONE = !BIG && T == 64;
+    constexpr bool ONE = T == 64;
     constexpr int ML = ONE ? 128 : 8 * T;
     __shared__ uint64_t khi[CAP];
     __shared__ klo_w klo[CAP];
@@ -133,10 +157,7 @@
     const int tid = threadIdx.x;
     const chunk_t ch = chunk_get(desc, c);
     if (ch.n == 0) return;
-    if (!BIG && ch.n > (uint32_t)CAP) {
-        if (tid == 0) biglist[atomicAdd(nbig, 1u)] = c;
-        return;
-    }
+    if (ch.n > (uint32_t)CAP) return;
     const uint32_t n = ch.n;
     uint64_t src = ch.base;
     if (rg.keys_r) { src = rg.desc_src[c]; keys = rg.keys_r; vals = rg.vals_r; }
@@ -348,33 +369,31 @@
         if (tid == 0) nbnd[c] = bcnt;
     }
 }
-template <int K, bool BIG, bool GR, int MM>
-constexpr int bl_prune_waves = BIG ? 1 : (K <= 48 && !GR) ? (MM <= 16 ? 8 : 7) : 6;
-template <int K, int CAP, int T, bool BIG, bool GR, int MM>
-__global__ void __launch_bounds__(T) __attribute__((amdgpu_waves_per_eu(bl_prune_waves<K, BIG, GR, MM>, 8))) bl_prune_kernel(const uint4* __restrict__ desc, uint32_t NB, bl_shard sh, bl_regions rg, const uint32_t* __restrict__ biglist_in,
+template <int K, int CAP, bool GR, int MM>
+constexpr int bl_prune_waves = CAP > MCAP ? 1 : CAP > SCAP ? 4 : (K <= 48 && !GR) ? (MM <= 16 ? 8 : 7) : 6;
+template <int K, int CAP, int T, bool LIST, bool GR, int MM>
+__global__ void __launch_bounds__(T) __attribute__((amdgpu_waves_per_eu(bl_prune_waves<K, CAP, GR, MM>, 8))) bl_prune_kernel(const uint4* __restrict__ desc, uint32_t NB, bl_shard sh, bl_regions rg, const uint32_t* __restrict__ list_in,
                                                      uint32_t nchunks, uint32_t cpw,
                                                      const snk_u128* __restrict__ keys, const uint64_t* __restrict__ vals,
                                                      uint32_t do_prune, uint8_t* __restrict__ ctx_out,
                                                      uint32_t* __restrict__ count_out, uint8_t* __restrict__ pend_out,
                                                      uint32_t* __restrict__ nbr_out, uint32_t* __restrict__ nbnd,
-                                                     uint32_t* __restrict__ biglist, uint32_t* __restrict__ nbig, const uint32_t* __restrict__ n_dev,
+                                                     const uint32_t* __restrict__ n_dev,
                                                      unsigned long long* __restrict__ gindex, uint64_t gmask, unsigned long long* __restrict__ spec) {
     __shared__ uint32_t shist[BL_SPEC_LDS];
     if (spec) {
         for (int j = threadIdx.x; j < BL_SPEC_LDS; j += T) shist[j] = 0;
         __syncthreads();
     }
-    if (BIG && n_dev) {
+    if constexpr (LIST) {
         const uint32_t nb = *n_dev;
         for (uint32_t w = blockIdx.x; w < nb; w += gridDim.x)
-            bl_prune_chunk<K, CAP, T, BIG, GR, MM>(biglist_in[w], desc, NB, sh, rg, keys, vals, do_prune, ctx_out, count_out, pend_out, nbr_out, nbnd, biglist, nbig, gindex, gmask,
-                                                   spec, shist);
+            bl_prune_chunk<K, CAP, T, GR, MM>(list_in[w], desc, NB, sh, rg, keys, vals, do_prune, ctx_out, count_out, pend_out, nbr_out, nbnd, gindex, gmask, spec, shist);
     } else {
         for (uint32_t r = 0; r < cpw; ++r) {
             const uint32_t w = blockIdx.x * cpw + r;
             if (w >= nchunks) break;
-            bl_prune_chunk<K, CAP, T, BIG, GR, MM>(BIG ? biglist_in[w] : w, desc, NB, sh, rg, keys, vals, do_prune, ctx_out, count_out, pend_out, nbr_out,
-                                           nbnd, biglist, nbig, gindex, gmask, spec, shist);
+            bl_prune_chunk<K, CAP, T, GR, MM>(w, desc, NB, sh, rg, keys, vals, do_prune, ctx_out, count_out, pend_out, nbr_out, nbnd, gindex, gmask, spec, shist);
         }
     }
     if (spec) {
@@ -473,8 +492,8 @@
     const unsigned long long* node_off;
     unsigned long long my_node_off;
 };
-template <int K, int CAP, int T, bool BIG, bool EMIT, bool DIST, bool GR>
-__global__ void __launch_bounds__(T) bl_frag_kernel(const uint4* __restrict__ desc, const uint32_t* __restrict__ biglist_in,
+template <int K, int CAP, int T, bool LIST, bool EMIT, bool DIST, bool GR>
+__global__ void __launch_bounds__(T) bl_frag_kernel(const uint4* __restrict__ desc, const uint32_t* __restrict__ list_in,
                                                     const snk_u128* __restrict__ keys, const uint8_t* __restrict__ ctx,
                                                     const uint8_t* __restrict__ pend, const uint32_t* __restrict__ nbr,
                                                     const uint32_t* __restrict__ rq, bl_dist_args da, uint32_t* __restrict__ nfrag,
@@ -490,9 +509,12 @@
     __shared__ uint64_t khi[ONEW ? 1 : CAP];
     __shared__ klo_w klo[ONEW ? 1 : CAP];
     __shared__ uint16_t nbL[2 * CAP];
-    typedef typename std::conditional<(CAP <= 256), uint32_t, uint64_t>::type wrec_t;
-    constexpr int FB = CAP <= 256 ? 10 : 16;
+    typedef typename std::conditional<(CAP <= 512), uint32_t, uint64_t>::type wrec_t;
+    constexpr int FB = CAP <= 256 ? 10 : CAP <= 512 ? 11 : 16;
+    constexpr int DB = CAP <= 512 ? 10 : 16;
     constexpr uint32_t FM = (1u << FB) - 1u;
+    constexpr uint32_t DM = (1u << DB) - 1u;
+    static_assert(2 * CAP <= (int)FM && CAP - 1 <= (int)DM && 2 * FB + DB <= 8 * (int)sizeof(wrec_t), "the ranking record holds every state and every hop count");
     __shared__ uint16_t lnk[2 * CAP];
     __shared__ wrec_t wr[2 * CAP];
     constexpr bool WIDE = (uint32_t)CAP * (uint32_t)K > 65535u;
@@ -502,10 +524,10 @@
     __shared__ uint8_t ctxL[CAP], pendL[CAP];
     __shared__ uint32_t fcnt, bcnt, changed;
     const int tid = threadIdx.x;
-    const uint32_t c = BIG ? biglist_in[blockIdx.x] : blockIdx.x;
+    const uint32_t c = LIST ? list_in[blockIdx.x] : blockIdx.x;
     const chunk_t ch = chunk_get(desc, c);
     if (ch.n == 0) return;
-    if (!BIG && ch.n > (uint32_t)CAP) return;
+    if (ch.n > (uint32_t)CAP) return;
     const uint32_t n = ch.n;
     const uint32_t c_foff = EMIT ? foff[c] : 0u;
     const uint64_t c_boff = EMIT ? boff[c] : 0ull;
@@ -582,8 +604,8 @@
         }
         lnk[s] = out;
         if (!EMIT) { if (out == NONE16) ++myterm; }
-        else if (out == NONE16) wr[s] = (wrec_t)FM | ((wrec_t)s << (2 * FB));
-        else wr[s] = (wrec_t)(out ^ 1u) | ((wrec_t)1 << FB) | ((wrec_t)(out ^ 1u) << (2 * FB));
+        else if (out == NONE16) wr[s] = (wrec_t)FM | ((wrec_t)s << (FB + DB));
+        else wr[s] = (wrec_t)(out ^ 1u) | ((wrec_t)1 << FB) | ((wrec_t)(out ^ 1u) << (FB + DB));
     }
     if (!EMIT) {
         if constexpr (ONEW) {
@@ -612,8 +634,8 @@
                 rr[q] = a0;
                 if (n1 != FM) {
                     const wrec_t a1 = wr[n1];
-                    const uint32_t d = (((uint32_t)(a0 >> FB) & FM) + ((uint32_t)(a1 >> FB) & FM)) & FM;
-                    rr[q] = (a1 & (wrec_t)FM) | ((wrec_t)d << FB) | (a1 & ((wrec_t)FM << (2 * FB)));
+                    const uint32_t d = (((uint32_t)(a0 >> FB) & DM) + ((uint32_t)(a1 >> FB) & DM)) & DM;
+                    rr[q] = (a1 & (wrec_t)FM) | ((wrec_t)d << FB) | (a1 & ((wrec_t)FM << (FB + DB)));
                     any = true;
                 }
             }
@@ -641,8 +663,8 @@
     }
     __syncthreads();
     auto w_next = [&](uint32_t st) -> uint32_t { return (uint32_t)wr[st] & FM; };
-    auto w_dist = [&](uint32_t st) -> uint32_t { return (uint32_t)(wr[st] >> FB) & FM; };
-    auto w_tail = [&](uint32_t st) -> uint32_t { return (uint32_t)(wr[st] >> (2 * FB)) & FM; };
+    auto w_dist = [&](uint32_t st) -> uint32_t { return (uint32_t)(wr[st] >> FB) & DM; };
+    auto w_tail = [&](uint32_t st) -> uint32_t { return (uint32_t)(wr[st] >> (FB + DB)) & FM; };
 
     auto half_link = [&](uint32_t s) -> unsigned long long {
         const uint32_t i = s >> 1, side = s & 1u;
@@ -829,9 +851,6 @@
 
 }
 
-constexpr int SCAP = 256, ST = 64;
-constexpr int BCAP = SNK_GRAPH_CHUNK_MAX, BT = 256;
-
 namespace {
 constexpr int QWORDS = 4;
 constexpr int QSPAN = 8 * QWORDS * TB;
@@ -927,23 +946,24 @@
     G_ALLOC(B->desc, uint4, (uint64_t)nchunks + 1);
     uint64_t* desc_src = nullptr;
     if (tab->keys_r) G_ALLOC(desc_src, uint64_t, (uint64_t)nchunks + 1);
-    SNK_HIP_TRY(snk_launch(bl_chunk_desc_kernel, snk_blocks(nchunks, 256), 256, 0, st, cs, nchunks, B->desc, tab->region_cap, desc_src));
     uint32_t *nbnd, *ctr;
+    G_ALLOC(B->midlist, uint32_t, n / SCAP + 2);
+    G_ALLOC(B->biglist, uint32_t, n / SCAP + 2);
+    G_ALLOC(ctr, uint32_t, 16);
+    SNK_HIP_TRY(hipMemsetAsync(ctr, 0, 64, st));
+    SNK_HIP_TRY(snk_launch(bl_chunk_desc_kernel, snk_blocks(nchunks, DESC_T), DESC_T, 0, st, cs, nchunks, B->desc, tab->region_cap, desc_src, B->midlist, B->biglist, ctr));
     G_ALLOC(B->ctx, uint8_t, n + 16);
     G_ALLOC(B->pend, uint8_t, n + 16);
     G_ALLOC(B->counts, uint32_t, n + 4);
     G_ALLOC(B->nbr, uint32_t, n + 2);
     G_ALLOC(B->rq, uint32_t, 2 * n + 2);
     G_ALLOC(nbnd, uint32_t, (uint64_t)nchunks + 1);
-    G_ALLOC(B->biglist, uint32_t, n / SCAP + 2);
-    G_ALLOC(ctr, uint32_t, 16);
     B->premote = nullptr;
     if (B->world > 1 || B->force_dist) {
         G_ALLOC(B->premote, uint8_t, n + 16);
         SNK_HIP_TRY(hipMemsetAsync(B->premote, 0, n + 16, st));
     }
     SNK_HIP_TRY(hipMemsetAsync(nbnd, 0, ((uint64_t)nchunks + 1) * 4, st));
-    SNK_HIP_TRY(hipMemsetAsync(ctr, 0, 64, st));
     bl_shard sh;
     sh.bucket_base = B->premote ? B->rank * B->NBl : 0u;
     sh.NBl = B->premote ? B->NBl : 0u;
@@ -970,14 +990,17 @@
     rg.keys_r = tab->keys_r; rg.vals_r = tab->vals_r; rg.desc_src = desc_src;
     rg.keys_dense = const_cast<snk_u128*>(tab->keys);
     const bool long_m = ctx->mlen == (uint32_t)SNK_M_LONG;
+    const uint32_t prune_mode = B->do_prune | (snk_opt_u32(ctx, SNK_OPT_bl_noclassify) ? 2u : 0u);
     SNK_HIP_TRY(snk_launch(long_m ? bl_prune_kernel<K, SCAP, ST, false, GR, SNK_M_LONG> : bl_prune_kernel<K, SCAP, ST, false, GR, SNK_M_OF(K)>, snk_blocks(nchunks, cpw), ST, 0, st, (const uint4*)B->desc, NBh, sh, rg,
-                           (const uint32_t*)nullptr, nchunks, cpw, tab->keys, tab->vals, B->do_prune | (snk_opt_u32(ctx, SNK_OPT_bl_noclassify) ? 2u : 0u), B->ctx, B->counts, B->pend, B->nbr, nbnd,
-                           B->biglist, ctr, (const uint32_t*)nullptr, index0, tg0 - 1, spec));
-    uint32_t h_nbig = 0;
-    SNK_HIP_TRY(hipMemcpyAsync(ctr + 1, ctr, 4, hipMemcpyDeviceToDevice, st));
+                           (const uint32_t*)nullptr, nchunks, cpw, tab->keys, tab->vals, prune_mode, B->ctx, B->counts, B->pend, B->nbr, nbnd,
+                           (const uint32_t*)nullptr, index0, tg0 - 1, spec));
+    uint32_t h_cls[2] = {0, 0};
+    SNK_HIP_TRY(snk_launch(long_m ? bl_prune_kernel<K, MCAP, MT, true, GR, SNK_M_LONG> : bl_prune_kernel<K, MCAP, MT, true, GR, SNK_M_OF(K)>, 4096, MT, 0, st, (const uint4*)B->desc, NBh, sh, rg,
+                           (const uint32_t*)B->midlist, 0u, 1u, tab->keys, tab->vals, prune_mode, B->ctx, B->counts, B->pend, B->nbr,
+                           nbnd, (const uint32_t*)ctr, index0, tg0 - 1, spec));
     SNK_HIP_TRY(snk_launch(long_m ? bl_prune_kernel<K, BCAP, BT, true, GR, SNK_M_LONG> : bl_prune_kernel<K, BCAP, BT, true, GR, SNK_M_OF(K)>, 2048, BT, 0, st, (const uint4*)B->desc, NBh, sh, rg,
-                           (const uint32_t*)B->biglist, 0u, 1u, tab->keys, tab->vals, B->do_prune | (snk_opt_u32(ctx, SNK_OPT_bl_noclassify) ? 2u : 0u), B->ctx, B->counts, B->pend, B->nbr,
-                           nbnd, B->biglist, ctr + 2, (const uint32_t*)(ctr + 1), index0, tg0 - 1, spec));
+                           (const uint32_t*)B->biglist, 0u, 1u, tab->keys, tab->vals, prune_mode, B->ctx, B->counts, B->pend, B->nbr,
+                           nbnd, (const uint32_t*)(ctr + 1), index0, tg0 - 1, spec));
     if (spec) SNK_HIP_TRY(snk_launch(bl_spec_fold_kernel, 1, BL_SPEC_LDS, 0, st, spec));
     if (tab->keys_r) {
         snk_ctx_release_block(ctx, tab->keys_r);
@@ -998,9 +1021,10 @@
     if (index0) SNK_HIP_TRY(hipMemcpyAsync(&h_gaveup, index0 + tg0, 8, hipMemcpyDeviceToHost, st));
     if (spec) SNK_HIP_TRY(hipMemcpyAsync(&h_spec_over, spec + BL_SPEC_OVER, 8, hipMemcpyDeviceToHost, st));
     SNK_HIP_TRY(hipMemcpyAsync(&h_bnd, d_sum, 8, hipMemcpyDeviceToHost, st));
-    SNK_HIP_TRY(hipMemcpyAsync(&h_nbig, ctr + 1, 4, hipMemcpyDeviceToHost, st));
+    SNK_HIP_TRY(hipMemcpyAsync(h_cls, ctr, 8, hipMemcpyDeviceToHost, st));
     SNK_HIP_TRY(snk_sync(st));
-    B->nbig = h_nbig;
+    B->nmid = h_cls[0];
+    B->nbig = h_cls[1];
     B->spec = spec;
     B->spec_over = h_spec_over != 0;
     B->n_boundary = h_bnd;
@@ -1027,7 +1051,7 @@
 static int bl_fragments_impl(snk_ctx* ctx, hipStream_t st, snk_bl_state* B, const bl_dist_args& da, snk_frag_out* out, char* err,
                              size_t errcap) {
     const snk_table* tab = B->tab;
-    const uint32_t nchunks = B->nchunks, h_nbig = B->nbig;
+    const uint32_t nchunks = B->nchunks, h_nmid = B->nmid, h_nbig = B->nbig;
     uint32_t *nfrag, *foff;
     uint64_t *nbases, *boff;
     G_ALLOC(nfrag, uint32_t, (uint64_t)nchunks + 1);
@@ -1041,10 +1065,16 @@
                            (const uint32_t*)nullptr, tab->keys, B->ctx, B->pend, B->nbr, B->rq, da, nfrag, (const uint32_t*)nullptr,
                            (const uint64_t*)nullptr, (uint32_t*)nullptr, (unsigned long long*)nullptr, (unsigned long long*)nullptr,
                            (uint64_t*)nullptr, (uint8_t*)nullptr, (uint32_t*)nullptr, (uint32_t*)nullptr, xp0));
-    SNK_HIP_TRY(snk_launch(bl_frag_kernel<K, BCAP, BT, true, false, DIST, GR>, h_nbig, BT, 0, st, (const uint4*)B->desc,
-                           (const uint32_t*)B->biglist, tab->keys, B->ctx, B->pend, B->nbr, B->rq, da, nfrag, (const uint32_t*)nullptr,
-                           (const uint64_t*)nullptr, (uint32_t*)nullptr, (unsigned long long*)nullptr, (unsigned long long*)nullptr,
-                           (uint64_t*)nullptr, (uint8_t*)nullptr, (uint32_t*)nullptr, (uint32_t*)nullptr, xp0));
+    if (h_nmid)
+        SNK_HIP_TRY(snk_launch(bl_frag_kernel<K, MCAP, MT, true, false, DIST, GR>, h_nmid, MT, 0, st, (const uint4*)B->desc,
+                               (const uint32_t*)B->midlist, tab->keys, B->ctx, B->pend, B->nbr, B->rq, da, nfrag, (const uint32_t*)nullptr,
+                               (const uint64_t*)nullptr, (uint32_t*)nullptr, (unsigned long long*)nullptr, (unsigned long long*)nullptr,
+                               (uint64_t*)nullptr, (uint8_t*)nullptr, (uint32_t*)nullptr, (uint32_t*)nullptr, xp0));
+    if (h_nbig)
+        SNK_HIP_TRY(snk_launch(bl_frag_kernel<K, BCAP, BT, true, false, DIST, GR>, h_nbig, BT, 0, st, (const uint4*)B->desc,
+                               (const uint32_t*)B->biglist, tab->keys, B->ctx, B->pend, B->nbr, B->rq, da, nfrag, (const uint32_t*)nullptr,
+                               (const uint64_t*)nullptr, (uint32_t*)nullptr, (unsigned long long*)nullptr, (unsigned long long*)nullptr,
+                               (uint64_t*)nullptr, (uint8_t*)nullptr, (uint32_t*)nullptr, (uint32_t*)nullptr, xp0));
     SNK_HIP_TRY(snk_launch(bl_chunk_bases_kernel, snk_blocks((uint64_t)nchunks + 1, TB), TB, 0, st, (const uint4*)B->desc, nfrag, nchunks,
                            (uint32_t)K, nbases));
     int rc;
@@ -1080,9 +1110,14 @@
         SNK_HIP_TRY(snk_launch(bl_frag_kernel<K, SCAP, ST, false, true, DIST, GR>, nchunks, ST, 0, st, (const uint4*)B->desc,
                                (const uint32_t*)nullptr, tab->keys, B->ctx, B->pend, B->nbr, B->rq, da, nfrag, foff, boff, out->nk, out->hl_self,
                                out->hl_nb, out->boff, out->bases, out->fgroup, out->sfrag, xp));
-        SNK_HIP_TRY(snk_launch(bl_frag_kernel<K, BCAP, BT, true, true, DIST, GR>, h_nbig, BT, 0, st, (const uint4*)B->desc,
-                               (const uint32_t*)B->biglist, tab->keys, B->ctx, B->pend, B->nbr, B->rq, da, nfrag, foff, boff, out->nk,
-                               out->hl_self, out->hl_nb, out->boff, out->bases, out->fgroup, out->sfrag, xp));
+        if (h_nmid)
+            SNK_HIP_TRY(snk_launch(bl_frag_kernel<K, MCAP, MT, true, true, DIST, GR>, h_nmid, MT, 0, st, (const uint4*)B->desc,
+                                   (const uint32_t*)B->midlist, tab->keys, B->ctx, B->pend, B->nbr, B->rq, da, nfrag, foff, boff, out->nk,
+                                   out->hl_self, out->hl_nb, out->boff, out->bases, out->fgroup, out->sfrag, xp));
+        if (h_nbig)
+            SNK_HIP_TRY(snk_launch(bl_frag_kernel<K, BCAP, BT, true, true, DIST, GR>, h_nbig, BT, 0, st, (const uint4*)B->desc,
+                                   (const uint32_t*)B->biglist, tab->keys, B->ctx, B->pend, B->nbr, B->rq, da, nfrag, foff, boff, out->nk,
+                                   out->hl_self, out->hl_nb, out->boff, out->bases, out->fgroup, out->sfrag, xp));
         SNK_HIP_TRY(hipMemcpyAsync(h_x, xcur, 16, hipMemcpyDeviceToHost, st));
         SNK_HIP_TRY(snk_sync(st));
         if (h_x[0] <= xf_cap && h_x[1] <= xb_cap) break;
@@ -1094,7 +1129,10 @@
     out->total_bases = h_B + h_x[1];
     out->n_local_circles = (uint32_t)h_x[0];
     ctx->last_bl_circles = h_x[0];
-    ctx->last_bl_big_chunks = h_nbig;
+    ctx->last_bl_big_chunks = h_nmid + h_nbig;
+    ctx->last_bl_classes[0] = nchunks - h_nmid - h_nbig;
+    ctx->last_bl_classes[1] = h_nmid;
+    ctx->last_bl_classes[2] = h_nbig;
     return SNK_OK;
 }
 
diff --git a/supernova_amd/csrc/snk_pipeline.hip b/supernova_amd/csrc/snk_pipeline.hip
--- a/supernova_amd/csrc/snk_pipeline.hip
+++ b/supernova_amd/csrc/snk_pipeline.hip
@@ -65,6 +65,7 @@
     snk_graph_out go;
     ctx->last_bl_attempts = ctx->last_bl_big_chunks = 0;
     ctx->last_bl_circles = 0;
+    ctx->last_bl_classes[0] = ctx->last_bl_classes[1] = ctx->last_bl_classes[2] = 0;
     if (local_graph) {
         snk_u128* keys_final = nullptr;
         rc = snk_local_graph(ctx, st, K, &tab, p->min_freq > 1 ? 1u : 0u, !(p->flags & SNK_F_NO_GRAPH),
diff --git a/supernova_amd/lib.py b/supernova_amd/lib.py
--- a/supernova_amd/lib.py
+++ b/supernova_amd/lib.py
@@ -391,6 +391,7 @@
         "snk_ctx_last_count_limit": (u32, [vp]),
         "snk_ctx_last_hbv_flood": (u32, [vp, P(u64), P(u64)]),
         "snk_ctx_last_local_graph": (u32, [vp, P(u64), P(u32)]),
+        "snk_ctx_last_chunk_classes": (None, [vp, P(u32)]),
         "snk_fasth_open": (C.c_int, [P(cp), u32, u32, u32, u32, u32, P(vp), cp, sz]),
         "snk_fasth_next": (C.c_int, [vp, P(SnkFasthBatch), cp, sz]),
         "snk_fasth_release": (None, [vp, P(SnkFasthBatch)]),
```
